# seanome/kmerseek

Measured on AMD Instinct MI355X. Metric: k-mers hashed+matched/sec, higher is better.
Workload: dtype u64

## Files before the change

include/kmerseek_amd.h:

```cpp
#ifndef KMERSEEK_AMD_H
#define KMERSEEK_AMD_H

#include <stddef.h>
#include <stdint.h>

#ifdef __cplusplus
extern "C" {
#endif

#define KS_ABI_VERSION 1

typedef enum ks_status {
    KS_OK = 0,
    KS_ERR_INVALID_MOLTYPE = 1,
    KS_ERR_INVALID_KSIZE = 2,
    KS_ERR_INVALID_RESIDUE = 3,
    KS_ERR_INVALID_ARG = 4,
    KS_ERR_OOM = 5,
    KS_ERR_HIP = 6,
    KS_ERR_NO_DEVICE = 7,
    KS_ERR_CAPACITY = 8,
    KS_ERR_INVALID_SCALED = 9
} ks_status;

typedef enum ks_moltype { KS_PROTEIN = 0, KS_DAYHOFF = 1, KS_HP = 2 } ks_moltype;

#define KS_SEED_DEFAULT 42ull
#define KS_MAX_KSIZE 128u

typedef struct ks_params {
    uint32_t ksize;
    uint32_t scaled;
    uint32_t moltype;
    uint32_t flags;
    uint64_t seed;
} ks_params;

typedef struct ks_ctx ks_ctx;
typedef struct ks_sketches ks_sketches;
typedef struct ks_index ks_index;
typedef struct ks_hits ks_hits;
typedef struct ks_kmerpos ks_kmerpos;
typedef struct ks_matchpos ks_matchpos;
typedef struct ks_regions ks_regions;
typedef struct ks_raligns ks_raligns;
typedef struct ks_cigars ks_cigars;
typedef struct ks_rscores ks_rscores;


uint32_t ks_abi_version(void);
const char *ks_status_string(int status);

int ks_moltype_from_string(const char *name, uint32_t *moltype_out);

uint64_t ks_max_hash(uint32_t scaled);

int ks_ctx_create(int device, void *hip_stream, ks_ctx **out);
void ks_ctx_destroy(ks_ctx *ctx);
const char *ks_last_error(const ks_ctx *ctx);
void *ks_ctx_stream(const ks_ctx *ctx);
int ks_ctx_synchronize(ks_ctx *ctx);
int ks_ctx_pool_stats(const ks_ctx *ctx, uint64_t *n_blocks, uint64_t *bytes_held, uint64_t *bytes_in_use,
                      uint64_t *n_mallocs);

int ks_ctx_sketch_stats(const ks_ctx *ctx, uint64_t out[4]);
int ks_ctx_search_stats(const ks_ctx *ctx, uint64_t out[5]);
int ks_ctx_fused_stats(const ks_ctx *ctx, uint64_t out[4]);
int ks_ctx_qfilter_stats(const ks_ctx *ctx, uint64_t out[2]);
int ks_ctx_reload_debug_env(ks_ctx *ctx);
int ks_debug_guard_selftest(const char *what);

int ks_dev_malloc(ks_ctx *ctx, uint64_t bytes, void **out);
int ks_dev_free(ks_ctx *ctx, void *ptr);
int ks_dev_upload(ks_ctx *ctx, void *dst_device, const void *src_host, uint64_t bytes);
int ks_dev_download(ks_ctx *ctx, void *dst_host, const void *src_device, uint64_t bytes);

int ks_host_alloc(ks_ctx *ctx, uint64_t bytes, void **out);
int ks_host_free(ks_ctx *ctx, void *ptr);


typedef struct ks_residue_error {
    uint32_t seq_index;
    uint32_t position;
    uint8_t residue;
} ks_residue_error;

int ks_validate_and_resolve(const uint8_t *seq, uint64_t len, int upper, uint64_t rng_seed,
                            uint8_t *out, uint64_t *out_len, ks_residue_error *err);


int ks_sketch_batch(ks_ctx *ctx, const uint8_t *residues, const uint64_t *seq_offsets,
                    uint32_t n_seqs, const ks_params *params, ks_sketches **out);

int ks_sketch_batch_device(ks_ctx *ctx, const uint8_t *d_residues, const uint64_t *d_seq_offsets,
                           uint32_t n_seqs, uint64_t n_residues, uint32_t max_seq_len,
                           const ks_params *params, ks_sketches **out);

int ks_sketch_queries_device(ks_ctx *ctx, const ks_index *index, const uint8_t *d_residues,
                             const uint64_t *d_seq_offsets, uint32_t n_seqs, uint64_t n_residues,
                             uint32_t max_seq_len, ks_sketches **out);

int ks_sketch_search_device(ks_ctx *ctx, const ks_index *index, const uint8_t *d_residues,
                            const uint64_t *d_seq_offsets, uint32_t n_seqs, uint64_t n_residues,
                            uint32_t max_seq_len, ks_sketches **sketches_out, ks_hits **hits_out);
int ks_sketch_search(ks_ctx *ctx, const ks_index *index, const uint8_t *residues, const uint64_t *seq_offsets,
                     uint32_t n_seqs, ks_sketches **sketches_out, ks_hits **hits_out);

uint32_t ks_sketches_n_seqs(const ks_sketches *s);
uint64_t ks_sketches_n_hashes(const ks_sketches *s);
uint64_t ks_sketches_n_windows(const ks_sketches *s);
int ks_sketches_has_postings(const ks_sketches *s);
void ks_sketches_params(const ks_sketches *s, ks_params *out);
const uint64_t *ks_sketches_device_offsets(const ks_sketches *s);
const uint64_t *ks_sketches_device_hashes(const ks_sketches *s);
const uint32_t *ks_sketches_device_abunds(const ks_sketches *s);
int ks_sketches_copy_to_host(ks_ctx *ctx, const ks_sketches *s, uint64_t *offsets,
                             uint64_t *hashes, uint32_t *abunds);
int ks_sketches_from_host(ks_ctx *ctx, const uint64_t *offsets, const uint64_t *hashes,
                          const uint32_t *abunds, uint32_t n_seqs, const ks_params *params,
                          ks_sketches **out);
int ks_sketches_union(ks_ctx *ctx, const ks_sketches *in, ks_sketches **out);
void ks_sketches_free(ks_sketches *s);


uint64_t ks_translate6_bound(uint64_t n_nt);
int ks_translate6_device(ks_ctx *ctx, const uint8_t *d_nt, const uint64_t *d_offsets, uint32_t n_seqs, uint64_t n_nt,
                         uint8_t *d_frames ,
                         uint64_t *d_frame_offsets , uint64_t *n_residues_out);
int ks_sketch_translated_device(ks_ctx *ctx, const uint8_t *d_nt, const uint64_t *d_offsets, uint32_t n_seqs, uint64_t n_nt,
                                uint32_t max_seq_len , const ks_params *params, ks_sketches **out);
int ks_sketch_translated(ks_ctx *ctx, const uint8_t *nt, const uint64_t *offsets, uint32_t n_seqs, const ks_params *params,
                         ks_sketches **out);
int ks_sketches_union_groups(ks_ctx *ctx, const ks_sketches *in, const uint32_t *group_offsets, uint32_t n_groups, ks_sketches **out);
uint32_t ks_debug_translate_chunk(void);
uint32_t ks_debug_union_rank_max(void);


#define KS_MASK_MAX_WINDOW 32
typedef struct ks_mask_opts { uint32_t window, k1_millibits, k2_millibits; } ks_mask_opts;
typedef struct ks_mask ks_mask;
typedef struct ks_segments ks_segments;
int ks_mask_device(ks_ctx *ctx, const uint8_t *d_residues, const uint64_t *d_seq_offsets, uint32_t n_seqs, uint64_t n_residues,
                   const ks_mask_opts *opts, ks_mask **out);
int ks_mask_batch(ks_ctx *ctx, const uint8_t *residues, const uint64_t *seq_offsets, uint32_t n_seqs, const ks_mask_opts *opts,
                  ks_mask **out);
uint32_t ks_mask_n_seqs(const ks_mask *m);
uint64_t ks_mask_n_residues(const ks_mask *m);
uint64_t ks_mask_n_masked(const ks_mask *m);
const uint8_t *ks_mask_device_mask(const ks_mask *m);
const uint32_t *ks_mask_device_masked_counts(const ks_mask *m);
int ks_mask_copy_to_host(ks_ctx *ctx, const ks_mask *m, uint8_t *mask, uint32_t *masked_counts);
void ks_mask_free(ks_mask *m);
int ks_mask_split_device(ks_ctx *ctx, const ks_mask *mask, const uint8_t *d_residues, const uint64_t *d_seq_offsets, uint32_t n_seqs,
                         uint64_t n_residues, uint32_t min_len, ks_segments **out);
uint64_t ks_segments_n_segs(const ks_segments *s);
uint64_t ks_segments_n_residues(const ks_segments *s);
uint32_t ks_segments_n_records(const ks_segments *s);
const uint32_t *ks_segments_device_seg_record(const ks_segments *s);
const uint32_t *ks_segments_device_seg_start(const ks_segments *s);
const uint64_t *ks_segments_device_seg_offsets(const ks_segments *s);
const uint8_t *ks_segments_device_residues(const ks_segments *s);
const uint32_t *ks_segments_device_group_offsets(const ks_segments *s);
int ks_segments_copy_to_host(ks_ctx *ctx, const ks_segments *s, uint32_t *seg_record, uint32_t *seg_start, uint64_t *seg_offsets,
                             uint8_t *residues, uint32_t *group_offsets);
void ks_segments_free(ks_segments *s);
int ks_sketch_masked_device(ks_ctx *ctx, const uint8_t *d_residues, const uint64_t *d_seq_offsets, uint32_t n_seqs, uint64_t n_residues,
                            uint32_t max_seq_len, const ks_params *params, const ks_mask_opts *opts, ks_sketches **out);
int ks_sketch_masked(ks_ctx *ctx, const uint8_t *residues, const uint64_t *seq_offsets, uint32_t n_seqs, const ks_params *params,
                     const ks_mask_opts *opts, ks_sketches **out);
int ks_kmer_positions_masked_device(ks_ctx *ctx, const uint8_t *d_residues, const uint64_t *d_seq_offsets, uint32_t n_seqs,
                                    uint64_t n_residues, const ks_params *params, const ks_mask_opts *opts, ks_kmerpos **out);
uint32_t ks_debug_mask_chunk(void);


int ks_kmer_positions(ks_ctx *ctx, const uint8_t *residues, const uint64_t *seq_offsets,
                      uint32_t n_seqs, const ks_params *params, ks_kmerpos **out);
int ks_kmer_positions_device(ks_ctx *ctx, const uint8_t *d_residues, const uint64_t *d_seq_offsets, uint32_t n_seqs,
                             uint64_t n_residues, const ks_params *params, ks_kmerpos **out);
uint64_t ks_kmerpos_count(const ks_kmerpos *p);
void ks_kmerpos_params(const ks_kmerpos *p, ks_params *out);
int ks_kmerpos_copy_to_host(ks_ctx *ctx, const ks_kmerpos *p, uint32_t *seq, uint32_t *start,
                            uint64_t *hash);
void ks_kmerpos_free(ks_kmerpos *p);


int ks_index_build(ks_ctx *ctx, const ks_sketches *targets, ks_index **out);
uint32_t ks_index_n_targets(const ks_index *ix);
uint64_t ks_index_n_postings(const ks_index *ix);
void ks_index_free(ks_index *ix);

int ks_search(ks_ctx *ctx, const ks_index *index, const ks_sketches *queries, ks_hits **out);
uint64_t ks_hits_count(const ks_hits *h);
uint64_t ks_hits_n_pair_instances(const ks_hits *h);
int ks_hits_partition_path(const ks_hits *h);
int ks_hits_bucket_posting_bytes(const ks_hits *h);
int ks_hits_copy_to_host(ks_ctx *ctx, const ks_hits *h, uint32_t *qid, uint32_t *tid,
                         uint32_t *intersect, uint64_t *n_weighted);
const uint32_t *ks_hits_device_qid(const ks_hits *h);
const uint32_t *ks_hits_device_tid(const ks_hits *h);
const uint32_t *ks_hits_device_intersect(const ks_hits *h);
const uint64_t *ks_hits_device_n_weighted(const ks_hits *h);
int ks_hits_copy_to_device(ks_ctx *ctx, const ks_hits *h, uint32_t qid_base, uint32_t tid_base, uint32_t *d_qid,
                           uint32_t *d_tid, uint32_t *d_intersect, uint64_t *d_n_weighted);
int ks_hits_pack64_to_device(ks_ctx *ctx, const ks_hits *h, uint32_t qid_base, uint32_t tid_base, int qbits, int tbits,
                             uint64_t *d_packed, uint32_t *d_esc_row, uint32_t *d_esc_intersect, uint64_t *d_esc_n_weighted,
                             uint32_t *d_n_esc, uint32_t esc_cap);
int ks_hits_unpack64_device(ks_ctx *ctx, const uint64_t *d_packed, uint64_t n, int qbits, int tbits, uint32_t *d_qid,
                            uint32_t *d_tid, uint32_t *d_intersect, uint64_t *d_n_weighted);
int ks_hits_merge_by_qid_device(ks_ctx *ctx, const uint32_t *d_qid, const uint32_t *d_tid, const uint32_t *d_intersect,
                                const uint64_t *d_n_weighted, const uint64_t *block_rows, uint32_t n_blocks, uint32_t n_queries,
                                uint32_t *d_out_qid, uint32_t *d_out_tid, uint32_t *d_out_intersect, uint64_t *d_out_n_weighted);
void ks_hits_free(ks_hits *h);


#define KS_SEARCH_ABUND_STATS 1u
typedef struct ks_search_opts {
    uint32_t flags;
    uint32_t reserved;
// ... 565 lines not shown
```

kmerseek_amd/_lib.py:

```python
from __future__ import annotations

import ctypes as C
import os
import sys

HERE = os.path.dirname(os.path.abspath(__file__))
SO_PATH = os.environ.get("KMERSEEK_AMD_LIB") or os.path.join(HERE, "libkmerseek_amd.so")

KS_OK = 0
KS_ERR_INVALID_MOLTYPE = 1
KS_ERR_INVALID_KSIZE = 2
KS_ERR_INVALID_RESIDUE = 3
KS_ERR_INVALID_ARG = 4
KS_ERR_OOM = 5
KS_ERR_HIP = 6
KS_ERR_NO_DEVICE = 7
KS_ERR_CAPACITY = 8
KS_ERR_INVALID_SCALED = 9

KS_PROTEIN, KS_DAYHOFF, KS_HP = 0, 1, 2
KS_SEED_DEFAULT = 42


class ks_params(C.Structure):
# ... 10 lines not shown

class ks_search_opts(C.Structure):
    _fields_ = [("flags", C.c_uint32), ("reserved", C.c_uint32), ("min_containment", C.c_double)]


class ks_matchpos_opts(C.Structure):
    _fields_ = [("flags", C.c_uint32), ("reserved", C.c_uint32), ("max_pairs", C.c_uint64)]


class ks_regions_opts(C.Structure):
    _fields_ = [("flags", C.c_uint32), ("min_kmers", C.c_uint32), ("max_gap", C.c_uint32), ("reserved", C.c_uint32)]


KS_RSCORE_ALPHABET = 28
KS_RSCORE_EXTEND = 1


class ks_rscore_opts(C.Structure):
    _fields_ = [("flags", C.c_uint32), ("x_drop", C.c_uint32), ("matrix", C.POINTER(C.c_int8)), ("reserved", C.c_uint64)]


KS_RALIGN_MAX_BAND = 31
KS_RALIGN_MAX_GAP_COST = 255
KS_RALIGN_MAX_X_DROP = 1 << 20


class ks_ralign_opts(C.Structure):
    _fields_ = [("matrix", C.POINTER(C.c_int8)), ("band", C.c_uint32), ("gap_open", C.c_uint32), ("gap_extend", C.c_uint32),
                ("x_drop", C.c_uint32), ("flags", C.c_uint32)]


KS_RTRACE_EQX = 1


class ks_rtrace_opts(C.Structure):
    _fields_ = [("flags", C.c_uint32), ("reserved", C.c_uint32), ("max_scratch_bytes", C.c_uint64)]


KS_RCULL_NONE = 0xFFFFFFFF
KS_RCULL_MIN_SCORE = 1


class ks_rcull_opts(C.Structure):
    _fields_ = [("overlap_pct", C.c_uint32), ("max_per_row", C.c_uint32), ("min_score", C.c_int64), ("flags", C.c_uint32),
                ("reserved", C.c_uint32)]


KS_RCHAIN_NONE = 0xFFFFFFFF


class ks_rchain_opts(C.Structure):
    _fields_ = [("max_gap", C.c_uint32), ("max_overlap", C.c_uint32), ("link_cost", C.c_uint32), ("skew_cost", C.c_uint32),
                ("overlap_cost", C.c_uint32), ("flags", C.c_uint32), ("reserved", C.c_uint32 * 2)]


KS_FFOLD_NONE = 0xFFFFFFFF


class ks_ffold_opts(C.Structure):
    _fields_ = [("flags", C.c_uint32), ("reserved", C.c_uint32 * 3)]


KS_RSTITCH_EQX = 1
KS_RSTITCH_MAX_FILL = 4096


class ks_rstitch_opts(C.Structure):
    _fields_ = [("max_fill", C.c_uint32), ("flags", C.c_uint32), ("max_scratch_bytes", C.c_uint64), ("reserved", C.c_uint32 * 2)]


KS_CIGAR_FSHIFT = 3
KS_FSTITCH_MAX_COST = 65536


class ks_fstitch_opts(C.Structure):
    _fields_ = [("max_fill", C.c_uint32), ("flags", C.c_uint32), ("frameshift_cost", C.c_uint32), ("reserved", C.c_uint32),
                ("max_scratch_bytes", C.c_uint64)]


KS_PILEUP_QUERY, KS_PILEUP_TARGET, KS_PILEUP_PROFILE = 0, 1, 1


class ks_pileup_opts(C.Structure):
    _fields_ = [("flags", C.c_uint32), ("side", C.c_uint32), ("reserved", C.c_uint64)]


KS_ASTATS_NO_COMPOSITION, KS_ASTATS_PAIRWISE, KS_ASTATS_ALLOW_UNGAPPED = 1, 2, 4
KS_ASTATS_ROW_REGULAR, KS_ASTATS_ROW_FALLBACK, KS_ASTATS_ROW_SKIPPED = 0, 1, 2
KS_ASTATS_MAX_SEQ_LEN = 1 << 20


class ks_astats_opts(C.Structure):
    _fields_ = [("flags", C.c_uint32), ("length_adjust", C.c_uint32), ("matrix", C.POINTER(C.c_int8)), ("lambda_", C.c_double),
                ("K", C.c_double), ("background", C.POINTER(C.c_double)), ("ratio_min", C.c_double), ("ratio_max", C.c_double),
                ("db_residues", C.c_uint64), ("db_seqs", C.c_uint64), ("reserved", C.c_uint64)]


class ks_signif_opts(C.Structure):
    _fields_ = [("flags", C.c_uint32), ("reserved", C.c_uint32)]


KS_BEST_INTERSECT, KS_BEST_TARGET_CONTAINMENT, KS_BEST_MAX_CONTAINMENT, KS_BEST_JACCARD, KS_BEST_SCORE = 0, 1, 2, 3, 4


class ks_best_opts(C.Structure):
    _fields_ = [("rank_by", C.c_uint32), ("k", C.c_uint32), ("flags", C.c_uint32), ("reserved", C.c_uint32)]


class ks_cluster_opts(C.Structure):
    _fields_ = [("similarity", C.c_uint32), ("n_nodes", C.c_uint32), ("threshold", C.c_double), ("flags", C.c_uint32),
                ("reserved", C.c_uint32)]


KS_GREEDY_ASSIGN_FIRST, KS_GREEDY_ASSIGN_BEST = 0, 1


class ks_greedy_opts(C.Structure):
    _fields_ = [("similarity", C.c_uint32), ("n_nodes", C.c_uint32), ("threshold", C.c_double), ("assign", C.c_uint32),
                ("flags", C.c_uint32)]


class ks_gather_opts(C.Structure):
    _fields_ = [("min_unique", C.c_uint32), ("max_results", C.c_uint32), ("flags", C.c_uint32), ("reserved", C.c_uint32)]


KS_MASK_MAX_WINDOW = 32


class ks_mask_opts(C.Structure):
    _fields_ = [("window", C.c_uint32), ("k1_millibits", C.c_uint32), ("k2_millibits", C.c_uint32)]


class ks_kernel_time(C.Structure):
    _fields_ = [("name", C.c_char * 48), ("launches", C.c_uint64), ("total_ms", C.c_double)]


_vp = C.c_void_p
_u8p = C.POINTER(C.c_uint8)
_u32p = C.POINTER(C.c_uint32)
_u64p = C.POINTER(C.c_uint64)
_pp = C.POINTER(C.c_void_p)
_parp = C.POINTER(ks_params)

SIGNATURES = {
    "ks_abi_version": (C.c_uint32, []),
    "ks_status_string": (C.c_char_p, [C.c_int]),
    "ks_moltype_from_string": (C.c_int, [C.c_char_p, _u32p]),
    "ks_max_hash": (C.c_uint64, [C.c_uint32]),
    "ks_ctx_create": (C.c_int, [C.c_int, _vp, _pp]),
    "ks_ctx_destroy": (None, [_vp]),
    "ks_last_error": (C.c_char_p, [_vp]),
    "ks_ctx_stream": (_vp, [_vp]),
    "ks_ctx_synchronize": (C.c_int, [_vp]),
    "ks_ctx_sketch_stats": (C.c_int, [_vp, C.POINTER(C.c_uint64 * 4)]),
    "ks_ctx_search_stats": (C.c_int, [_vp, C.POINTER(C.c_uint64 * 5)]),
    "ks_ctx_fused_stats": (C.c_int, [_vp, C.POINTER(C.c_uint64 * 4)]),
    "ks_ctx_qfilter_stats": (C.c_int, [_vp, C.POINTER(C.c_uint64 * 2)]),
    "ks_ctx_reload_debug_env": (C.c_int, [_vp]),
    "ks_debug_guard_selftest": (C.c_int, [C.c_char_p]),
    "ks_host_alloc": (C.c_int, [_vp, C.c_uint64, _pp]),
    "ks_host_free": (C.c_int, [_vp, _vp]),
    "ks_dev_malloc": (C.c_int, [_vp, C.c_uint64, _pp]),
    "ks_dev_free": (C.c_int, [_vp, _vp]),
    "ks_dev_upload": (C.c_int, [_vp, _vp, _vp, C.c_uint64]),
    "ks_dev_download": (C.c_int, [_vp, _vp, _vp, C.c_uint64]),
    "ks_ctx_pool_stats": (C.c_int, [_vp, _u64p, _u64p, _u64p, _u64p]),
    "ks_validate_and_resolve": (C.c_int, [C.c_char_p, C.c_uint64, C.c_int, C.c_uint64, C.c_char_p, _u64p,
                                          C.POINTER(ks_residue_error)]),
    "ks_sketch_batch": (C.c_int, [_vp, _vp, _vp, C.c_uint32, _parp, _pp]),
    "ks_sketch_batch_device": (C.c_int, [_vp, _vp, _vp, C.c_uint32, C.c_uint64, C.c_uint32, _parp, _pp]),
    "ks_sketch_queries_device": (C.c_int, [_vp, _vp, _vp, _vp, C.c_uint32, C.c_uint64, C.c_uint32, _pp]),
    "ks_sketch_search_device": (C.c_int, [_vp, _vp, _vp, _vp, C.c_uint32, C.c_uint64, C.c_uint32, _pp, _pp]),
    "ks_sketch_search": (C.c_int, [_vp, _vp, _vp, _vp, C.c_uint32, _pp, _pp]),
    "ks_sketches_has_postings": (C.c_int, [_vp]),
    "ks_sketches_n_seqs": (C.c_uint32, [_vp]),
    "ks_sketches_n_hashes": (C.c_uint64, [_vp]),
    "ks_sketches_n_windows": (C.c_uint64, [_vp]),
    "ks_sketches_params": (None, [_vp, _parp]),
    "ks_sketches_device_offsets": (_vp, [_vp]),
    "ks_sketches_device_hashes": (_vp, [_vp]),
    "ks_sketches_device_abunds": (_vp, [_vp]),
    "ks_sketches_copy_to_host": (C.c_int, [_vp, _vp, _vp, _vp, _vp]),
    "ks_sketches_from_host": (C.c_int, [_vp, _vp, _vp, _vp, C.c_uint32, _parp, _pp]),
    "ks_sketches_union": (C.c_int, [_vp, _vp, _pp]),
    "ks_sketches_free": (None, [_vp]),
    "ks_translate6_bound": (C.c_uint64, [C.c_uint64]),
    "ks_translate6_device": (C.c_int, [_vp, _vp, _vp, C.c_uint32, C.c_uint64, _vp, _vp, _u64p]),
    "ks_sketch_translated_device": (C.c_int, [_vp, _vp, _vp, C.c_uint32, C.c_uint64, C.c_uint32, _parp, _pp]),
    "ks_sketch_translated": (C.c_int, [_vp, _vp, _vp, C.c_uint32, _parp, _pp]),
    "ks_sketches_union_groups": (C.c_int, [_vp, _vp, _u32p, C.c_uint32, _pp]),
    "ks_debug_translate_chunk": (C.c_uint32, []),
    "ks_debug_union_rank_max": (C.c_uint32, []),
    "ks_mask_device": (C.c_int, [_vp, _vp, _vp, C.c_uint32, C.c_uint64, C.POINTER(ks_mask_opts), _pp]),
    "ks_mask_batch": (C.c_int, [_vp, _vp, _vp, C.c_uint32, C.POINTER(ks_mask_opts), _pp]),
    "ks_mask_n_seqs": (C.c_uint32, [_vp]),
    "ks_mask_n_residues": (C.c_uint64, [_vp]),
    "ks_mask_n_masked": (C.c_uint64, [_vp]),
    "ks_mask_device_mask": (_vp, [_vp]),
    "ks_mask_device_masked_counts": (_vp, [_vp]),
    "ks_mask_copy_to_host": (C.c_int, [_vp, _vp, _vp, _vp]),
    "ks_mask_free": (None, [_vp]),
    "ks_mask_split_device": (C.c_int, [_vp, _vp, _vp, _vp, C.c_uint32, C.c_uint64, C.c_uint32, _pp]),
    "ks_segments_n_segs": (C.c_uint64, [_vp]),
    "ks_segments_n_residues": (C.c_uint64, [_vp]),
    "ks_segments_n_records": (C.c_uint32, [_vp]),
    "ks_segments_device_seg_record": (_vp, [_vp]),
    "ks_segments_device_seg_start": (_vp, [_vp]),
    "ks_segments_device_seg_offsets": (_vp, [_vp]),
    "ks_segments_device_residues": (_vp, [_vp]),
    "ks_segments_device_group_offsets": (_vp, [_vp]),
    "ks_segments_copy_to_host": (C.c_int, [_vp, _vp, _vp, _vp, _vp, _vp, _vp]),
    "ks_segments_free": (None, [_vp]),
    "ks_sketch_masked_device": (C.c_int, [_vp, _vp, _vp, C.c_uint32, C.c_uint64, C.c_uint32, _parp, C.POINTER(ks_mask_opts), _pp]),
    "ks_sketch_masked": (C.c_int, [_vp, _vp, _vp, C.c_uint32, _parp, C.POINTER(ks_mask_opts), _pp]),
    "ks_kmer_positions_masked_device": (C.c_int, [_vp, _vp, _vp, C.c_uint32, C.c_uint64, _parp, C.POINTER(ks_mask_opts), _pp]),
    "ks_debug_mask_chunk": (C.c_uint32, []),
    "ks_kmer_positions": (C.c_int, [_vp, _vp, _vp, C.c_uint32, _parp, _pp]),
    "ks_kmer_positions_device": (C.c_int, [_vp, _vp, _vp, C.c_uint32, C.c_uint64, _parp, _pp]),
    "ks_kmerpos_count": (C.c_uint64, [_vp]),
    "ks_kmerpos_params": (None, [_vp, _parp]),
    "ks_kmerpos_copy_to_host": (C.c_int, [_vp, _vp, _vp, _vp, _vp]),
    "ks_kmerpos_free": (None, [_vp]),
    "ks_index_build": (C.c_int, [_vp, _vp, _pp]),
    "ks_index_n_targets": (C.c_uint32, [_vp]),
    "ks_index_n_postings": (C.c_uint64, [_vp]),
    "ks_index_free": (None, [_vp]),
    "ks_search": (C.c_int, [_vp, _vp, _vp, _pp]),
    "ks_hits_count": (C.c_uint64, [_vp]),
    "ks_hits_n_pair_instances": (C.c_uint64, [_vp]),
    "ks_hits_partition_path": (C.c_int, [_vp]),
    "ks_hits_bucket_posting_bytes": (C.c_int, [_vp]),
    "ks_hits_copy_to_host": (C.c_int, [_vp, _vp, _vp, _vp, _vp, _vp]),
    "ks_hits_device_qid": (_vp, [_vp]),
    "ks_hits_device_tid": (_vp, [_vp]),
    "ks_hits_device_intersect": (_vp, [_vp]),
    "ks_hits_device_n_weighted": (_vp, [_vp]),
    "ks_hits_copy_to_device": (C.c_int, [_vp, _vp, C.c_uint32, C.c_uint32, _vp, _vp, _vp, _vp]),
    "ks_hits_pack64_to_device": (C.c_int, [_vp, _vp, C.c_uint32, C.c_uint32, C.c_int, C.c_int, _vp, _vp, _vp, _vp, _vp, C.c_uint32]),
    "ks_hits_unpack64_device": (C.c_int, [_vp, _vp, C.c_uint64, C.c_int, C.c_int, _vp, _vp, _vp, _vp]),
    "ks_hits_merge_by_qid_device": (C.c_int, [_vp, _vp, _vp, _vp, _vp, C.POINTER(C.c_uint64), C.c_uint32, C.c_uint32, _vp, _vp, _vp, _vp]),
    "ks_hits_free": (None, [_vp]),
    "ks_search_ex": (C.c_int, [_vp, _vp, _vp, C.POINTER(ks_search_opts), _pp]),
    "ks_sketch_search_device_ex": (C.c_int, [_vp, _vp, _vp, _vp, C.c_uint32, C.c_uint64, C.c_uint32, C.POINTER(ks_search_opts), _pp,
                                             _pp]),
    "ks_sketch_search_ex": (C.c_int, [_vp, _vp, _vp, _vp, C.c_uint32, C.POINTER(ks_search_opts), _pp, _pp]),
    "ks_hits_has_abund_stats": (C.c_int, [_vp]),
    "ks_hits_device_median2": (_vp, [_vp]),
    "ks_hits_device_abund_ss": (_vp, [_vp]),
    "ks_hits_copy_abund_stats_to_host": (C.c_int, [_vp, _vp, _vp, _vp]),
    "ks_match_positions": (C.c_int, [_vp, _vp, _vp, _vp, C.POINTER(ks_matchpos_opts), _pp]),
    "ks_matchpos_n_rows": (C.c_uint64, [_vp]),
    "ks_matchpos_n_pairs": (C.c_uint64, [_vp]),
    "ks_matchpos_n_slices": (C.c_uint32, [_vp]),
    "ks_matchpos_device_row_offsets": (_vp, [_vp]),
    "ks_matchpos_device_q_start": (_vp, [_vp]),
    "ks_matchpos_device_t_start": (_vp, [_vp]),
    "ks_matchpos_device_q_lo": (_vp, [_vp]),
    "ks_matchpos_device_q_hi": (_vp, [_vp]),
    "ks_matchpos_device_t_lo": (_vp, [_vp]),
    "ks_matchpos_device_t_hi": (_vp, [_vp]),
    "ks_matchpos_copy_to_host": (C.c_int, [_vp, _vp, _vp, _vp, _vp, _vp, _vp, _vp, _vp]),
    "ks_matchpos_free": (None, [_vp]),
    "ks_match_regions": (C.c_int, [_vp, _vp, C.POINTER(ks_regions_opts), _pp]),
    "ks_regions_n_rows": (C.c_uint64, [_vp]),
    "ks_regions_n_regions": (C.c_uint64, [_vp]),
    "ks_regions_n_slices": (C.c_uint32, [_vp]),
    "ks_regions_device_row_offsets": (_vp, [_vp]),
    "ks_regions_device_q_start": (_vp, [_vp]),
    "ks_regions_device_t_start": (_vp, [_vp]),
    "ks_regions_device_length": (_vp, [_vp]),
    "ks_regions_device_n_kmers": (_vp, [_vp]),
    "ks_regions_device_covered": (_vp, [_vp]),
    "ks_regions_copy_to_host": (C.c_int, [_vp, _vp, _vp, _vp, _vp, _vp, _vp, _vp]),
    "ks_regions_free": (None, [_vp]),
    "ks_regions_score": (C.c_int, [_vp, _vp, _vp, _vp, _vp, C.c_uint32, C.c_uint64, _vp, _vp, C.c_uint32, C.c_uint64,
                                   C.POINTER(ks_rscore_opts), _pp]),
    "ks_rscores_n_rows": (C.c_uint64, [_vp]),
    "ks_rscores_n_regions": (C.c_uint64, [_vp]),
    "ks_rscores_device_row_offsets": (_vp, [_vp]),
    "ks_rscores_device_q_start": (_vp, [_vp]),
    "ks_rscores_device_t_start": (_vp, [_vp]),
    "ks_rscores_device_length": (_vp, [_vp]),
    "ks_rscores_device_score": (_vp, [_vp]),
    "ks_rscores_device_identities": (_vp, [_vp]),
    "ks_rscores_device_positives": (_vp, [_vp]),
    "ks_rscores_device_core_identities": (_vp, [_vp]),
    "ks_rscores_copy_to_host": (C.c_int, [_vp, _vp, _vp, _vp, _vp, _vp, _vp, _vp, _vp, _vp]),
    "ks_rscores_free": (None, [_vp]),
    "ks_debug_rscore_step": (C.c_uint32, []),
    "ks_regions_align": (C.c_int, [_vp, _vp, _vp, _vp, _vp, C.c_uint32, C.c_uint64, _vp, _vp, C.c_uint32, C.c_uint64,
                                   C.POINTER(ks_ralign_opts), _pp]),
    "ks_raligns_n_rows": (C.c_uint64, [_vp]),
    "ks_raligns_n_regions": (C.c_uint64, [_vp]),
    "ks_raligns_device_row_offsets": (_vp, [_vp]),
    "ks_raligns_device_q_start": (_vp, [_vp]),
    "ks_raligns_device_q_length": (_vp, [_vp]),
    "ks_raligns_device_t_start": (_vp, [_vp]),
    "ks_raligns_device_t_length": (_vp, [_vp]),
    "ks_raligns_device_score": (_vp, [_vp]),
    "ks_raligns_device_identities": (_vp, [_vp]),
    "ks_raligns_device_positives": (_vp, [_vp]),
    "ks_raligns_device_gap_opens": (_vp, [_vp]),
    "ks_raligns_device_gaps": (_vp, [_vp]),
    "ks_raligns_device_aln_length": (_vp, [_vp]),
    "ks_raligns_copy_to_host": (C.c_int, [_vp] * 13),
    "ks_raligns_free": (None, [_vp]),
    "ks_debug_ralign_chunk": (C.c_uint32, []),
# ... 262 lines not shown
```

kmerseek_amd/csrc/ks_common.h:

```cpp
#pragma once

#include <hip/hip_runtime.h>

#include <cstdint>
#include <cstdio>
#include <cstring>
#include <functional>
#include <initializer_list>
#include <new>
#include <stdexcept>
#include <string>
#include <vector>

#include "../../include/kmerseek_amd.h"

typedef uint8_t u8;
typedef uint16_t u16;
typedef uint32_t u32;
typedef uint64_t u64;
typedef int32_t i32;
typedef int64_t i64;

#define KS_WAVE 64

struct ks_pool_block {
    void *ptr;
    size_t size;
    bool in_use;
};

struct ks_timer_slot {
    hipEvent_t a, b;
    int name_id;
};

struct ks_copy_engine;

#define KS_DBG_LIST(X)                                                                                                   \
    X(STAGED_H2D) X(PLAIN_COPIES) X(PAIRS_LSD) X(MSD_LDS_CAP) X(SCAN_3PASS) X(INDEX_LSD) X(JOIN_FP) X(FP_COARSEN)        \
    X(PAIR_LIMIT) X(PBITS_MAX) X(RECORD_BITS) X(ONE_CURSOR) X(JOIN_SEGS) X(JOIN_SEG_CAP) X(JOIN_SPARSE)                \
    X(NO_ROWS_HINT) X(ROWS_TICKET) X(FORCE_ROWS_TICKET_RETRY) X(FORCE_TICKET_RETRY) X(NO_PLAN) X(NO_COMPACT) X(SPAN)      \
    X(NO_PACK) X(PLAN_SYNC) X(TILE_R) X(OUT_CAP) X(POOL_CAP) X(THROW) X(QCAP) X(LOOKBACK_SKIP) X(SYNC_API) X(POSTINGS12) X(POSTINGS10) X(NO_DEFER) X(BUCKET) X(JOIN_SPLIT) X(SUBSHIFT) X(MATCHPOS_ROW_BITS) X(SIGNIF_WAVE_ROWS) X(BEST_PATH) X(REGIONS_ROW_BITS) X(QFILTER) X(QFILTER_OCC) X(CLUSTER_PATH) X(GATHER_PATH) X(GREEDY_PATH) X(UNION_PATH) X(AGG_CAP) X(ROWS_PATH) X(CULL_PATH) X(CHAIN_PATH) X(COMP_PATH) X(PILEUP_PATH)
enum ks_dbg_id {
#define KS_DBG_ENUM(n) KS_DBG_##n,
    KS_DBG_LIST(KS_DBG_ENUM)
#undef KS_DBG_ENUM
    KS_DBG_COUNT
};
struct ks_debug {
    bool set[KS_DBG_COUNT];
    char val[KS_DBG_COUNT][32];
};
void ks_debug_load(ks_debug *d);

struct ks_ctx {
    int device = 0;
    ks_copy_engine *copy = nullptr;
    hipStream_t stream = nullptr;
    bool own_stream = false;
    int n_cus = 256;
    ks_debug dbg;
    u64 pool_cap = 0;
    std::string err;
    std::vector<ks_pool_block> pool;
    u64 pool_mallocs = 0;
    int timing = 0;
    std::vector<std::string> t_names;
    std::vector<u64> t_launches;
    std::vector<double> t_ms;
    std::vector<ks_timer_slot> t_pending;
    std::vector<std::pair<hipEvent_t, hipEvent_t>> t_free;
    bool t_open = false;
    u64 *h_pin = nullptr;
    u64 pair_cap_hint = 0;
    u64 rows_hint = 0;
    bool sketch_use_ticket = false;
    u64 sketch_ticket_fallbacks = 0, sketch_compact_fallbacks = 0, sketch_cap_fallbacks = 0;
    bool rows_use_ticket = false; u64 rows_ticket_fallbacks = 0;
    u64 fused_deferred = 0, fused_redos = 0;
    u64 fused_aggregated = 0;
    u64 join_retries = 0;
    double rows_mult = 0.0;
    u64 agg_used = 0, agg_overflows = 0, agg_oflow_rows = 0;
    bool qfilter_pays = true;
    u64 qfilter_seen = 0, qfilter_dropped = 0;
    u64 qf_last_seen = 0, qf_last_kept = 0;
    u64 join_table = 0, fused_table_joined = 0;
    unsigned long long *scan_ring = nullptr;
    u32 *scan_ticket = nullptr;
    u32 scan_ticket_base = 0;
    u8 *d_lut = nullptr;
    unsigned long long *h_flag = nullptr;
    unsigned long long wait_seq = 0;
};

int ks_stream_wait(ks_ctx *ctx);
#define KS_FETCH_MAX 4
struct ks_fetch_seg {
    const void *src;
    u32 *dst;
    u32 rows, row_words, src_stride;
};
static inline ks_fetch_seg ks_fetch_words(const void *src, void *dst, u32 n_words32) { return ks_fetch_seg{src, (u32 *)dst, 1u, n_words32, n_words32}; }
int ks_stream_wait_fetch(ks_ctx *ctx, const ks_fetch_seg *segs, int n);

void *ks_pool_alloc(ks_ctx *ctx, size_t bytes);
void ks_pool_free(ks_ctx *ctx, void *ptr);
void ks_pool_trim(ks_ctx *ctx);

int ks_fail(ks_ctx *ctx, int status, const char *fmt, ...);
static inline const char *ks_dbg(const ks_ctx *ctx, int id) { return (ctx && ctx->dbg.set[id]) ? ctx->dbg.val[id] : nullptr; }

int ks_guard_fail(ks_ctx *ctx, int status, const char *what) noexcept;
void ks_guard_enter(ks_ctx *ctx);
template <typename F>
static inline int ks_guard(ks_ctx *ctx, F &&body) noexcept {
    try {
        ks_guard_enter(ctx);
        return body();
    } catch (const std::bad_alloc &) {
        return ks_guard_fail(ctx, KS_ERR_OOM, "out of host memory (std::bad_alloc)");
    } catch (const std::exception &e) {
        return ks_guard_fail(ctx, KS_ERR_HIP, e.what());
    } catch (...) {
        return ks_guard_fail(ctx, KS_ERR_HIP, "unknown exception");
    }
}

void ks_timer_begin(ks_ctx *ctx, const char *name);
void ks_timer_end(ks_ctx *ctx);

#define KS_HIP(ctx, expr)                                                                          \
    do {                                                                                           \
        hipError_t e__ = (expr);                                                                   \
        if (e__ != hipSuccess)                                                                     \
            return ks_fail(ctx, KS_ERR_HIP, "%s failed: %s (%s:%d)", #expr, hipGetErrorString(e__), \
                           __FILE__, __LINE__);                                                    \
    } while (0)

#define KS_TRY(expr)                        \
    do {                                    \
        int s__ = (expr);                   \
        if (s__ != KS_OK) return s__;       \
    } while (0)

#define KS_LAUNCH(ctx, name, kernel, grid, block, ...)                                   \
    do {                                                                                 \
        ks_timer_begin(ctx, name);                                                       \
        hipLaunchKernelGGL(kernel, dim3(grid), dim3(block), 0, (ctx)->stream, __VA_ARGS__); \
        ks_timer_end(ctx);                                                               \
        KS_HIP(ctx, hipGetLastError());                                                  \
    } while (0)

template <typename T>
static inline int ks_alloc(ks_ctx *ctx, T **out, size_t count) {
    void *p = ks_pool_alloc(ctx, (count ? count : 1) * sizeof(T));
    if (!p) return KS_ERR_OOM;
    *out = (T *)p;
    return KS_OK;
}

struct ks_scratch {
    ks_ctx *ctx;
    void *blk[16];
    int n = 0;
    explicit ks_scratch(ks_ctx *c) : ctx(c) {}
    ks_scratch(const ks_scratch &) = delete;
    ~ks_scratch() { for (int i = 0; i < n; i++) ks_pool_free(ctx, blk[i]); }
    template <typename T> int alloc(T **out, size_t count) {
        if (n == 16) return ks_fail(ctx, KS_ERR_HIP, "internal error: scratch table full");
        KS_TRY(ks_alloc(ctx, out, count));
        blk[n++] = *out;
        return KS_OK;
    }
    void free(void *p) { if (forget(p)) ks_pool_free(ctx, p); }
    template <typename T> T *keep(T *p) { forget(p); return p; }
    bool forget(void *p) {
        for (int i = 0; p && i < n; i++)
            if (blk[i] == p) { blk[i] = blk[--n]; return true; }
        return false;
    }
};

struct ks_ctl {
    u64 *dev = nullptr;
    u64 *host = nullptr;
    u32 n_words = 0;
    int init(ks_ctx *ctx, ks_scratch &sc, u32 pin_slot, u32 n_bad, u32 n_count) {
        n_words = n_bad + n_count;
        host = ctx->h_pin + pin_slot;
        KS_TRY(sc.alloc(&dev, n_words));
        KS_HIP(ctx, hipMemsetAsync(dev, 0xff, n_bad * sizeof(u64), ctx->stream));
        KS_HIP(ctx, hipMemsetAsync(dev + n_bad, 0, n_count * sizeof(u64), ctx->stream));
        return KS_OK;
    }
    unsigned long long *words() const { return (unsigned long long *)dev; }
    u32 *low32(u32 i) const { return (u32 *)(dev + i); }
    ks_fetch_seg fetch() const { return ks_fetch_words(dev, host, 2 * n_words); }
    u64 operator[](u32 i) const { return host[i]; }
    bool bad(u32 i) const { return host[i] != ~0ULL; }
};

template <typename T>
struct ks_result {
    T *obj = nullptr;
    T **out;
    void (*free_fn)(T *);
    ks_result(ks_ctx *ctx, T **out_, void (*f)(T *)) : out(out_), free_fn(f) {
        *out = nullptr;
        obj = new T();
        obj->ctx = ctx;
    }
    ks_result(const ks_result &) = delete;
    ~ks_result() {
        if (!obj) return;
        (void)hipStreamSynchronize(obj->ctx->stream);
        free_fn(obj);
    }
    T *operator->() const { return obj; }
    operator T *() const { return obj; }
    int commit() { *out = obj; obj = nullptr; return KS_OK; }
};

struct ks_column { void *dst; const void *src; size_t bytes; };
int ks_copy_d2h(ks_ctx *ctx, void *dst_host, const void *src_device, size_t bytes);
static inline int ks_columns_to_host(ks_ctx *ctx, const ks_column *cols, size_t n) {
    KS_HIP(ctx, hipSetDevice(ctx->device));
    for (const ks_column *c = cols; c < cols + n; c++)
        if (c->dst && c->bytes) KS_TRY(ks_copy_d2h(ctx, c->dst, c->src, c->bytes));
    KS_HIP(ctx, hipStreamSynchronize(ctx->stream));
// ... 602 lines not shown
```

kmerseek_amd/csrc/ks_ctx.hip:

```cpp
#include <cstdarg>
#include <algorithm>

#include "ks_common.h"

int ks_fail(ks_ctx *ctx, int status, const char *fmt, ...) {
    char buf[512];
    va_list ap;
    va_start(ap, fmt);
    vsnprintf(buf, sizeof buf, fmt, ap);
    va_end(ap);
    if (ctx) {
        try { ctx->err = buf; } catch (...) { }
    }
    return status;
}

extern "C" uint32_t ks_abi_version(void) { return KS_ABI_VERSION; }


bool ks_same_params(const ks_params &a, const ks_params &b) {
    return a.ksize == b.ksize && a.scaled == b.scaled && a.moltype == b.moltype && a.seed == b.seed && a.flags == b.flags;
}
int ks_params_check_same(ks_ctx *ctx, const char *pass, const char *noun, const ks_params &a, const ks_params &b) {
    if (ks_same_params(a, b)) return KS_OK;
// ... 18 lines not shown
}

static void build_luts(u8 *lut) {
    for (int m = 0; m < 3; m++)
        for (int b = 0; b < 256; b++) {
            u8 c = (b >= 'a' && b <= 'z') ? (u8)(b - 32) : (u8)b;
            u8 e = c;
            if (m == KS_DAYHOFF) {
                switch (c) {
                case 'C': e = 'a'; break;
                case 'A': case 'G': case 'P': case 'S': case 'T': e = 'b'; break;
                case 'D': case 'E': case 'N': case 'Q': e = 'c'; break;
                case 'H': case 'K': case 'R': e = 'd'; break;
                case 'I': case 'L': case 'M': case 'V': e = 'e'; break;
                case 'F': case 'W': case 'Y': e = 'f'; break;
                default: e = 'X';
                }
            } else if (m == KS_HP) {
                switch (c) {
                case 'A': case 'F': case 'G': case 'I': case 'L': case 'M': case 'P': case 'V':
                case 'W': case 'Y': e = 'h'; break;
                case 'N': case 'C': case 'S': case 'T': case 'D': case 'E': case 'R': case 'H':
                case 'K': case 'Q': e = 'p'; break;
                default: e = 'X';
                }
            }
            lut[m * 256 + b] = e;
        }
}

void ks_debug_load(ks_debug *d) {
    static const char *const names[KS_DBG_COUNT] = {
#define KS_DBG_NAME(n) "KS_DEBUG_" #n,
        KS_DBG_LIST(KS_DBG_NAME)
#undef KS_DBG_NAME
    };
    for (int i = 0; i < KS_DBG_COUNT; i++) {
        const char *v = getenv(names[i]);
        d->set[i] = v != nullptr;
        d->val[i][0] = 0;
        if (v) { strncpy(d->val[i], v, sizeof d->val[i] - 1); d->val[i][sizeof d->val[i] - 1] = 0; }
    }
}
static void debug_apply(ks_ctx *ctx) {
    ks_debug_load(&ctx->dbg);
    const char *cap = ks_dbg(ctx, KS_DBG_POOL_CAP);
    ctx->pool_cap = cap ? strtoull(cap, nullptr, 10) : 0;
}
extern "C" int ks_ctx_reload_debug_env(ks_ctx *ctx) {
    if (!ctx) return KS_ERR_INVALID_ARG;
    debug_apply(ctx);
    return KS_OK;
}

int ks_guard_fail(ks_ctx *ctx, int status, const char *what) noexcept {
    if (ctx) {
        try {
            ctx->err.assign(status == KS_ERR_OOM ? "" : "internal error: ");
            ctx->err.append(what ? what : "?");
        } catch (...) {
        }
    }
    return status;
}
void ks_guard_enter(ks_ctx *ctx) {
    const char *t = ks_dbg(ctx, KS_DBG_THROW);
    if (!t) return;
    if (!strcmp(t, "bad_alloc")) throw std::bad_alloc();
    if (!strcmp(t, "runtime")) throw std::runtime_error("KS_DEBUG_THROW");
    if (!strcmp(t, "other")) throw 42;
}

extern "C" int ks_debug_guard_selftest(const char *what) {
    return ks_guard(nullptr, [&]() -> int {
        if (what && !strcmp(what, "bad_alloc")) { std::vector<char> v; v.reserve((size_t)-1 / 2); }
        if (what && !strcmp(what, "runtime")) throw std::runtime_error("selftest");
        if (what && !strcmp(what, "other")) throw 42;
        return KS_OK;
    });
}

extern "C" int ks_ctx_create(int device, void *hip_stream, ks_ctx **out) {
    if (!out) return KS_ERR_INVALID_ARG;
    *out = nullptr;
    int n = 0;
    if (hipGetDeviceCount(&n) != hipSuccess || n <= 0) return KS_ERR_NO_DEVICE;
    if (device < 0 || device >= n) return KS_ERR_INVALID_ARG;
    ks_ctx *ctx = new (std::nothrow) ks_ctx();
    if (!ctx) return KS_ERR_OOM;
    ctx->device = device;
    try { ctx->err.reserve(640); ctx->pool.reserve(256); } catch (...) { delete ctx; return KS_ERR_OOM; }
    debug_apply(ctx);
    if (hipSetDevice(device) != hipSuccess) { delete ctx; return KS_ERR_HIP; }
    hipDeviceProp_t prop;
    if (hipGetDeviceProperties(&prop, device) == hipSuccess) ctx->n_cus = prop.multiProcessorCount;
    if (hip_stream) {
        ctx->stream = (hipStream_t)hip_stream;
    } else {
        if (hipStreamCreateWithFlags(&ctx->stream, hipStreamNonBlocking) != hipSuccess) { delete ctx; return KS_ERR_HIP; }
        ctx->own_stream = true;
    }
    if (hipHostMalloc((void **)&ctx->h_pin, KS_PIN_WORDS * sizeof(u64), hipHostMallocCoherent) != hipSuccess) { delete ctx; return KS_ERR_HIP; }
    if (hipHostMalloc((void **)&ctx->h_flag, 64, hipHostMallocCoherent) != hipSuccess) { (void)hipGetLastError(); ctx->h_flag = nullptr; }
    else *ctx->h_flag = 0;
    if (hipMalloc((void **)&ctx->d_lut, 3 * 256) != hipSuccess) { delete ctx; return KS_ERR_OOM; }
    u8 lut[768];
    build_luts(lut);
    if (hipMemcpy(ctx->d_lut, lut, sizeof lut, hipMemcpyHostToDevice) != hipSuccess) { delete ctx; return KS_ERR_HIP; }
    *out = ctx;
    return KS_OK;
}

extern "C" void ks_ctx_destroy(ks_ctx *ctx) {
    if (!ctx) return;
    (void)hipSetDevice(ctx->device);
    (void)hipStreamSynchronize(ctx->stream);
    ks_copy_engine_destroy(ctx);
    for (auto &t : ctx->t_pending) { (void)hipEventDestroy(t.a); (void)hipEventDestroy(t.b); }
    for (auto &t : ctx->t_free) { (void)hipEventDestroy(t.first); (void)hipEventDestroy(t.second); }
    for (auto &b : ctx->pool) (void)hipFree(b.ptr);
    if (ctx->d_lut) (void)hipFree(ctx->d_lut);
    if (ctx->h_pin) (void)hipHostFree(ctx->h_pin);
    if (ctx->h_flag) (void)hipHostFree(ctx->h_flag);
    if (ctx->scan_ring) (void)hipFree(ctx->scan_ring);
    if (ctx->scan_ticket) (void)hipFree(ctx->scan_ticket);
    if (ctx->own_stream) (void)hipStreamDestroy(ctx->stream);
    delete ctx;
}

extern "C" const char *ks_last_error(const ks_ctx *ctx) { return ctx ? ctx->err.c_str() : "no context"; }
extern "C" void *ks_ctx_stream(const ks_ctx *ctx) { return ctx ? (void *)ctx->stream : nullptr; }
extern "C" int ks_ctx_synchronize(ks_ctx *ctx) {
    return ks_guard(ctx, [&]() -> int {
    if (!ctx) return KS_ERR_INVALID_ARG;
    KS_HIP(ctx, hipStreamSynchronize(ctx->stream));
    return KS_OK;
    });
}

extern "C" int ks_ctx_pool_stats(const ks_ctx *ctx, uint64_t *n_blocks, uint64_t *bytes_held, uint64_t *bytes_in_use,
                                 uint64_t *n_mallocs) {
    return ks_guard((ks_ctx *)ctx, [&]() -> int {
    if (!ctx) return KS_ERR_INVALID_ARG;
    u64 held = 0, used = 0;
    for (auto &b : ctx->pool) { held += b.size; if (b.in_use) used += b.size; }
    if (n_blocks) *n_blocks = ctx->pool.size();
    if (bytes_held) *bytes_held = held;
    if (bytes_in_use) *bytes_in_use = used;
    if (n_mallocs) *n_mallocs = ctx->pool_mallocs;
    return KS_OK;
    });
}

extern "C" int ks_ctx_sketch_stats(const ks_ctx *ctx, uint64_t out[4]) {
    return ks_guard((ks_ctx *)ctx, [&]() -> int {
    if (!ctx || !out) return KS_ERR_INVALID_ARG;
    out[0] = ctx->sketch_ticket_fallbacks; out[1] = ctx->sketch_use_ticket ? 1 : 0;
    out[2] = ctx->sketch_compact_fallbacks; out[3] = ctx->sketch_cap_fallbacks;
    return KS_OK;
    });
}

extern "C" int ks_ctx_search_stats(const ks_ctx *ctx, uint64_t out[5]) {
    return ks_guard((ks_ctx *)ctx, [&]() -> int {
    if (!ctx || !out) return KS_ERR_INVALID_ARG;
    out[0] = ctx->join_retries; out[1] = ctx->rows_ticket_fallbacks;
    out[2] = ctx->agg_used; out[3] = ctx->agg_overflows;
    out[4] = ctx->join_table;
    return KS_OK;
    });
}

extern "C" int ks_ctx_qfilter_stats(const ks_ctx *ctx, uint64_t out[2]) {
    return ks_guard((ks_ctx *)ctx, [&]() -> int {
    if (!ctx || !out) return KS_ERR_INVALID_ARG;
    out[0] = ctx->qfilter_seen; out[1] = ctx->qfilter_dropped;
    return KS_OK;
    });
}

extern "C" int ks_ctx_fused_stats(const ks_ctx *ctx, uint64_t out[4]) {
    return ks_guard((ks_ctx *)ctx, [&]() -> int {
    if (!ctx || !out) return KS_ERR_INVALID_ARG;
    out[0] = ctx->fused_deferred; out[1] = ctx->fused_redos; out[2] = ctx->fused_aggregated;
    out[3] = ctx->fused_table_joined;
    return KS_OK;
    });
}

extern "C" int ks_dev_malloc(ks_ctx *ctx, uint64_t bytes, void **out) {
    return ks_guard(ctx, [&]() -> int {
    if (!ctx || !out) return KS_ERR_INVALID_ARG;
    KS_HIP(ctx, hipSetDevice(ctx->device));
    if (hipMalloc(out, bytes ? bytes : 256) != hipSuccess) { (void)hipGetLastError(); return ks_fail(ctx, KS_ERR_OOM, "hipMalloc(%llu) failed", (unsigned long long)bytes); }
    return KS_OK;
    });
}
extern "C" int ks_dev_free(ks_ctx *ctx, void *ptr) {
    return ks_guard(ctx, [&]() -> int {
    if (!ctx) return KS_ERR_INVALID_ARG;
    KS_HIP(ctx, hipStreamSynchronize(ctx->stream));
    KS_HIP(ctx, hipFree(ptr));
    return KS_OK;
    });
}
extern "C" int ks_dev_upload(ks_ctx *ctx, void *dst, const void *src, uint64_t bytes) {
    return ks_guard(ctx, [&]() -> int {
    if (!ctx || (bytes && (!dst || !src))) return KS_ERR_INVALID_ARG;
    KS_HIP(ctx, hipSetDevice(ctx->device));
    KS_TRY(ks_copy_h2d(ctx, dst, src, (size_t)bytes));
    KS_HIP(ctx, hipStreamSynchronize(ctx->stream));
    return KS_OK;
    });
}
extern "C" int ks_dev_download(ks_ctx *ctx, void *dst, const void *src, uint64_t bytes) {
    return ks_guard(ctx, [&]() -> int {
    if (!ctx || (bytes && (!dst || !src))) return KS_ERR_INVALID_ARG;
    KS_HIP(ctx, hipSetDevice(ctx->device));
    KS_TRY(ks_copy_d2h(ctx, dst, src, (size_t)bytes));
    KS_HIP(ctx, hipStreamSynchronize(ctx->stream));
    return KS_OK;
    });
}

__global__ void k_host_stamp(unsigned long long *flag, unsigned long long seq) {
    __hip_atomic_store(flag, seq, __ATOMIC_RELEASE, __HIP_MEMORY_SCOPE_SYSTEM);
}
struct ks_fetch_args { ks_fetch_seg seg[KS_FETCH_MAX]; int n; };
__global__ __launch_bounds__(256) void k_host_report(ks_fetch_args F, unsigned long long *flag, unsigned long long seq) {
    for (int s = 0; s < F.n; s++) {
        const ks_fetch_seg g = F.seg[s];
        const u32 total = g.rows * g.row_words;
        for (u32 i = threadIdx.x; i < total; i += blockDim.x) {
            const u32 r = i / g.row_words, c = i - r * g.row_words;
            const u32 v = __hip_atomic_load((const u32 *)g.src + (size_t)r * g.src_stride + c, __ATOMIC_RELAXED, __HIP_MEMORY_SCOPE_AGENT);
            __hip_atomic_store(g.dst + i, v, __ATOMIC_RELAXED, __HIP_MEMORY_SCOPE_SYSTEM);
        }
    }
    __threadfence_system();
    __syncthreads();
    if (threadIdx.x == 0) __hip_atomic_store(flag, seq, __ATOMIC_RELEASE, __HIP_MEMORY_SCOPE_SYSTEM);
}

static int stream_wait_poll(ks_ctx *ctx, unsigned long long seq);

int ks_stream_wait_fetch(ks_ctx *ctx, const ks_fetch_seg *segs, int n) {
    if (n > KS_FETCH_MAX) return ks_fail(ctx, KS_ERR_INVALID_ARG, "too many fetch segments");
    if (!ctx->h_flag || ks_dbg(ctx, KS_DBG_SYNC_API)) {
        for (int i = 0; i < n; i++) {
            const ks_fetch_seg &g = segs[i];
            if (g.rows == 1 || g.src_stride == g.row_words)
                KS_HIP(ctx, hipMemcpyAsync(g.dst, g.src, (size_t)g.rows * g.row_words * sizeof(u32), hipMemcpyDeviceToHost, ctx->stream));
            else
                KS_HIP(ctx, hipMemcpy2DAsync(g.dst, (size_t)g.row_words * sizeof(u32), g.src, (size_t)g.src_stride * sizeof(u32),
                                            (size_t)g.row_words * sizeof(u32), g.rows, hipMemcpyDeviceToHost, ctx->stream));
        }
        KS_HIP(ctx, hipStreamSynchronize(ctx->stream));
        return KS_OK;
    }
    ks_fetch_args F;
    memset(&F, 0, sizeof F);
    for (int i = 0; i < n; i++) F.seg[i] = segs[i];
    F.n = n;
    const unsigned long long seq = ++ctx->wait_seq;
    hipLaunchKernelGGL(k_host_report, dim3(1), dim3(256), 0, ctx->stream, F, ctx->h_flag, seq);
    if (hipGetLastError() != hipSuccess) return ks_fail(ctx, KS_ERR_HIP, "k_host_report launch failed");
    return stream_wait_poll(ctx, seq);
}

int ks_stream_wait(ks_ctx *ctx) {
    if (!ctx->h_flag || ks_dbg(ctx, KS_DBG_SYNC_API)) {
        KS_HIP(ctx, hipStreamSynchronize(ctx->stream));
        return KS_OK;
    }
    const unsigned long long seq = ++ctx->wait_seq;
    hipLaunchKernelGGL(k_host_stamp, dim3(1), dim3(1), 0, ctx->stream, ctx->h_flag, seq);
    if (hipGetLastError() != hipSuccess) { KS_HIP(ctx, hipStreamSynchronize(ctx->stream)); return KS_OK; }
    return stream_wait_poll(ctx, seq);
}

static int stream_wait_poll(ks_ctx *ctx, unsigned long long seq) {
    for (unsigned spins = 1;; spins++) {
        if (__atomic_load_n(ctx->h_flag, __ATOMIC_ACQUIRE) == seq) return KS_OK;
        if ((spins & 0xfffu) == 0) {
            const hipError_t q = hipStreamQuery(ctx->stream);
            if (q == hipSuccess) {
                if (__atomic_load_n(ctx->h_flag, __ATOMIC_ACQUIRE) == seq) return KS_OK;
                KS_HIP(ctx, hipStreamSynchronize(ctx->stream));
                return KS_OK;
            }
            if (q != hipErrorNotReady) return ks_fail(ctx, KS_ERR_HIP, "stream failed: %s", hipGetErrorString(q));
            if (spins > (1u << 26)) { KS_HIP(ctx, hipStreamSynchronize(ctx->stream)); return KS_OK; }
        }
#if defined(__x86_64__)
        __builtin_ia32_pause();
#endif
    }
}

static size_t pool_class(size_t bytes) {
    if (bytes <= 4096) return (bytes + 255) & ~(size_t)255;
    const int e = 63 - __builtin_clzll((unsigned long long)(bytes - 1));
    const size_t step = (size_t)1 << (e - 2);
    return (bytes + step - 1) & ~(step - 1);
}

void *ks_pool_alloc(ks_ctx *ctx, size_t bytes) {
    if (bytes == 0) bytes = 256;
    const size_t want = pool_class(bytes);
    for (size_t i = 0; i < ctx->pool.size(); i++) {
        auto &b = ctx->pool[i];
// ... 239 lines not shown
```

kmerseek_amd/csrc/ks_sketch.hip:

```cpp
#include "ks_tile.h"

#define SK_MED_MAX (SK_TILE - 16)
#define SK_NR 8
static const u32 sk_r_cand_host[SK_NR] = {2544, 2800, 3056, 3312, 3568, 3824, 3952, 4016};
#ifndef SK_MINW
#define SK_MINW 6
#endif
#define SK_NFLAG (SK_TILE / 32)
#ifndef SK_LB_WAVES
#define SK_LB_WAVES 1
#endif
#define SK_C3MAX 32u
#define SK_QB_CAP 128u

#ifdef SK_STAMP
#define SK_STAMP_SLOTS 4096
__device__ unsigned long long sk_stamp_acc[SK_STAMP_SLOTS][16];
#define SK_STAMP_AT(i) do { if (threadIdx.x == 0) { unsigned long long t_ = clock64(); \
    atomicAdd(&sk_stamp_acc[blockIdx.x % SK_STAMP_SLOTS][i], t_ - sk_t_prev); sk_t_prev = clock64(); } } while (0)
extern "C" void ks_debug_read_stamps(unsigned long long *out, int reset) {
    static unsigned long long host[SK_STAMP_SLOTS][16];
    (void)hipMemcpyFromSymbol(host, HIP_SYMBOL(sk_stamp_acc), sizeof host);
    for (int i = 0; i < 16; i++) { out[i] = 0; for (int s = 0; s < SK_STAMP_SLOTS; s++) out[i] += host[s][i]; }
    if (reset) { memset(host, 0, sizeof host); (void)hipMemcpyToSymbol(HIP_SYMBOL(sk_stamp_acc), host, sizeof host); }
}
#elif defined(SK_STOP_AFTER)
#define SK_STAMP_AT(i) do { if ((i) == SK_STOP_AFTER) return; } while (0)
#else
#define SK_STAMP_AT(i) do { } while (0)
#endif

KS_DEV bool sk_deferred(u64 start, u64 len, u32 R, u32 span) { return start % R + len > span - 16; }
KS_DEV u32 sk_div(u32 x, u32 d, u32 rcp) { return d == 1 ? x : __umulhi(x, rcp); }

KS_DEV u32 sk_wave_totals_scan(const u32 *smem, u32 lane, u32 wave_u , u32 *total) {
    constexpr u32 NW = SK_THREADS / 64;
    static_assert(NW <= 16, "one DPP row");
    u32 v = lane < NW ? smem[lane] : 0u;
    v += (u32)__builtin_amdgcn_update_dpp(0, (int)v, 0x111, 0xf, 0xf, true);
    v += (u32)__builtin_amdgcn_update_dpp(0, (int)v, 0x112, 0xf, 0xf, true);
    v += (u32)__builtin_amdgcn_update_dpp(0, (int)v, 0x114, 0xf, 0xf, true);
    if (NW > 8) v += (u32)__builtin_amdgcn_update_dpp(0, (int)v, 0x118, 0xf, 0xf, true);
    *total = (u32)__builtin_amdgcn_readlane((int)v, NW - 1);
    return wave_u ? (u32)__builtin_amdgcn_readlane((int)v, (int)wave_u - 1) : 0u;
}
KS_DEV u32 sk_block_excl_scan2(u32 a, u32 b, u32 *smem, u32 *total_a, u32 *excl_b) {
    const u32 lane = threadIdx.x & 63, wave = threadIdx.x >> 6;
    constexpr u32 NW = SK_THREADS / 64;
    const u32 ia = ks_wave_incl_scan(a), ib = ks_wave_incl_scan(b);
    if (lane == 63) { smem[wave] = ia; smem[NW + 1 + wave] = ib; }
    __syncthreads();
    const u32 wave_u = (u32)__builtin_amdgcn_readfirstlane((int)wave);
    u32 tot_b;
    const u32 base_a = sk_wave_totals_scan(smem, lane, wave_u, total_a);
    const u32 base_b = sk_wave_totals_scan(smem + NW + 1, lane, wave_u, &tot_b);
    *excl_b = base_b + ib - b;
    if (threadIdx.x == 0) smem[NW] = tot_b;
    return base_a + ia - a;
}

KS_DEV u32 sk_block_excl_scan1(u32 a, u32 *smem) {
    const u32 lane = threadIdx.x & 63, wave = threadIdx.x >> 6;
    const u32 ia = ks_wave_incl_scan(a);
    if (lane == 63) smem[wave] = ia;
    __syncthreads();
    u32 total;
    const u32 base = sk_wave_totals_scan(smem, lane, (u32)__builtin_amdgcn_readfirstlane((int)wave), &total);
    return base + ia - a;
}

KS_DEV u32 sk_digit(u64 h, u32 K, u32 kshift, u32 mask) {
    const u32 hi = (u32)(h >> 32);
    return (kshift ? (hi >> kshift) : __umulhi(hi, K)) & mask;
}

enum : u32 {
    SK_CTL_WINDOWS = 0, SK_CTL_MAX_LEN = 1,
    SK_CTL_N_PK_LONG = 2,
    SK_CTL_MED = 4, SK_CTL_LONG = 4 + SK_NR,
    SK_CTL_TICKET = 20,
    SK_CTL_CLS = 21,
    SK_CTL_PK_TILES = 22,
    SK_CTL_TOTAL = 23,
    SK_CTL_DROPS = 24,
    SK_CTL_LB_ROUNDS = 25,
    SK_CTL_DROPS_DEF = 26,
    SK_CTL_WORDS = 32,
    SK_CTL_CURSORS = SK_CTL_WORDS, SK_CTL_CURSOR_WORDS = 1024,
    SK_CTL_TILE_STATUS = SK_CTL_CURSORS + SK_CTL_CURSOR_WORDS,
};
static_assert(SK_CTL_LONG + SK_NR <= SK_CTL_TICKET && SK_CTL_LB_ROUNDS < SK_CTL_WORDS && SK_CTL_DROPS_DEF < SK_CTL_WORDS,
              "sketch control block layout");
static_assert(SK_CTL_WORDS <= KS_PIN_SKETCH_WORDS && SK_CTL_WORDS <= KS_PIN_SKETCH_SYNC_WORDS, "pinned slots of the sketch read-back");
enum : u32 { SK_ST_LOOKBACK = 1u, SK_ST_POSTINGS = 2u, SK_ST_COMPACT = 4u };
#define SK_BO_B(x) (((x) >> 12) & 0xfffu)
#define SK_BO_O(x) ((x) & 0xfffu)
#define SK_BO_S(x) ((x) >> 24)

struct sk_bounds {
    const u32 *loff;
    const u64 *goff;
    u64 g0;
    u32 s_first;
    bool in_lds;
    KS_DEV u32 at(u32 s) const {
        if (in_lds) return loff[s - s_first];
        u64 v = goff[s] - g0;
        return v > 0x7fffffffULL ? 0x7fffffffu : (u32)v;
    }
};

struct sk_seq {
    u32 s;
    u32 ls, le;
    u32 nw;
    u32 mul;
    bool ok;
};

KS_DEV void sk_load_seq(sk_seq &q, const sk_args &A, const sk_bounds &B, u32 s_end) {
    if (q.s >= s_end) { q.ok = false; q.ls = 0xffffffffu; q.le = 0xffffffffu; q.nw = 0; q.mul = 0; return; }
    q.ls = B.at(q.s);
    q.le = B.at(q.s + 1);
    const u32 len = q.le - q.ls;
    q.nw = (len >= A.k && q.le <= A.le_cap && len <= A.max_len_tile) ? (len - A.k + 1) : 0;
    q.mul = sk_bucket_mul(q.nw, A.sfix);
    q.ok = q.nw > 0;
}

KS_DEV u32 sk_place_window(const sk_args &A, u32 p, u64 h, sk_seq &q, const sk_bounds &B, u32 s_end, u32 *cnt) {
    while (q.s < s_end && p >= q.le) { q.s++; sk_load_seq(q, A, B, s_end); }
    const bool keep = q.ok && p >= q.ls && p + A.k <= q.le && h != 0 && h <= A.max_hash;
    u32 bo = 0xffffffffu;
    if (keep) {
        const u32 b = q.ls + __umulhi((u32)(h >> 32), q.mul);
        const u32 sh = (b & 1u) * 16u;
        const u32 o = (atomicAdd(&cnt[b >> 1], 1u << sh) >> sh) & 0xffffu;
        const u32 srel = q.s - B.s_first;
        bo = ((srel < 254u ? srel : 254u) << 24) | (b << 12) | o;
    }
    return bo;
}


#define PK_CHUNK 1024
#define PK_MAX_LEN (SK_MED_MAX - 16)

__global__ __launch_bounds__(64) void k_pack_walk(const u64 *offs, u32 n_seqs, u32 chunk ,
                                                  u32 *chunk_tiles , u32 *chunk_cnt) {
    __shared__ u64 lo_s[PK_CHUNK + 1];
    const u32 lane = threadIdx.x;
    const u32 c0 = blockIdx.x * chunk;
    const u32 n = (n_seqs - c0) < chunk ? (n_seqs - c0) : chunk;
    for (u32 i = lane; i <= n; i += 64) lo_s[i] = offs[c0 + i];
    __builtin_amdgcn_wave_barrier();
    u32 s = 0, nt = 0;
    while (s < n) {
        const u64 limit = (lo_s[s] & ~15ULL) + SK_MED_MAX;
        u32 lo = s, hi = n + 1;
        while (hi - lo > 1) {
            const u32 step = (hi - lo + 63) / 64;
            const u32 idx = lo + (lane + 1) * step;
            const bool ok = idx < hi && lo_s[idx] <= limit;
            const u64 m = __ballot(ok);
            const u32 good = m == ~0ULL ? 64u : (u32)__builtin_ctzll(~m);
            const u32 nlo = lo + good * step;
            const u32 nhi = lo + (good + 1) * step;
            lo = nlo < hi ? nlo : hi - 1;
            hi = nhi < hi ? nhi : hi;
        }
        u32 e = lo;
        if (e == s) e = s + 1;
        else if (e < n && lo_s[e + 1] - lo_s[e] > PK_MAX_LEN) e++;
        if (lane == 0) chunk_tiles[c0 + nt] = c0 + s;
        nt++;
        s = e;
    }
    if (lane == 0) chunk_cnt[blockIdx.x] = nt;
}

__global__ __launch_bounds__(256) void k_pack_fill(const u64 *offs, u32 n_seqs, u32 chunk, const u32 *chunk_tiles, const u32 *chunk_cnt, u32 n_chunks,
                                                   u32 *tile_first, u64 *tile_g0, u32 *n_tiles_out) {
    __shared__ u32 scan_smem[256 / 64 + 1];
    u32 part = 0;
    for (u32 c = threadIdx.x; c < blockIdx.x; c += 256) part += chunk_cnt[c];
    u32 total;
    (void)ks_block_excl_scan(part, scan_smem, &total);
    const u32 base = total, mine = chunk_cnt[blockIdx.x];
    for (u32 i = threadIdx.x; i < mine; i += 256) {
        const u32 sf = chunk_tiles[blockIdx.x * chunk + i];
        tile_first[base + i] = sf;
        tile_g0[base + i] = offs[sf] & ~15ULL;
    }
    if (blockIdx.x == n_chunks - 1 && threadIdx.x == 0) {
        tile_first[base + mine] = n_seqs;
        *n_tiles_out = base + mine;
    }
}

__global__ __launch_bounds__(256) void k_tile_plan(const u64 *offs, u32 n_seqs, u32 n_tiles, u32 R, u32 *tile_first) {
    const u32 t = blockIdx.x * blockDim.x + threadIdx.x;
    if (t > n_tiles) return;
    tile_first[t] = t == n_tiles ? n_seqs : ks_lower_bound_u64(offs, n_seqs, (u64)t * R);
}

template <int H, int NW, int KC>
KS_DEV void sk_cmp_half(const sk_args &A, const sk_bounds &B, sk_seq &q, const u64 *wl, u32 p0, bool active, u32 s_first, u32 s_end,
                        u32 lane, u64 *hlist, u8 *slist, u32 *cursor) {
    static_assert(NW == 4 || NW == 8, "a half or the whole of a thread's windows");
    u64 h[NW];
    u32 keep = 0, sr[2] = {0, 0};
    if (active) {
        sk_hash_windows<H, NW, KC>(h, wl, A.k, A.seed);
        if ((KC ? (u32)KC : A.k) >= SK_E) {
            const u32 srel = q.s - s_first;
#pragma unroll
            for (int i = 0; i < NW; i++)
                if ((p0 + H + i - q.ls) < q.nw && h[i] != 0 && h[i] <= A.max_hash) keep |= 1u << i;
            sr[0] = sr[1] = srel * 0x01010101u;
        } else {
#pragma unroll
            for (int i = 0; i < NW; i++) {
                const u32 p = p0 + H + i;
                while (q.s < s_end && p >= q.le) { q.s++; sk_load_seq(q, A, B, s_end); }
                if (q.ok && p >= q.ls && p + A.k <= q.le && h[i] != 0 && h[i] <= A.max_hash) {
                    keep |= 1u << i;
                    sr[i >> 2] |= (q.s - s_first) << (8 * (i & 3));
                }
            }
        }
    }
    const u32 nk = (u32)__popc(keep);
    const u32 incl = ks_wave_incl_scan(nk);
    const u32 wtot = (u32)__builtin_amdgcn_readlane((int)incl, 63);
    u32 wbase = 0;
    if (wtot) {
        if (lane == 0) wbase = atomicAdd(cursor, wtot);
        wbase = (u32)__builtin_amdgcn_readfirstlane((int)wbase);
    }
    u32 pos = wbase + incl - nk;
#pragma unroll
    for (int i = 0; i < NW; i++)
        if (keep & (1u << i)) {
            if (pos < SK_TILE) {
                hlist[pos] = h[i];
                slist[pos] = (u8)(sr[i >> 2] >> (8 * (i & 3)));
            }
            pos++;
        }
}

template <int MODE, int CMP, int KC>
KS_DEV void sk_tile_body(const sk_args &A, const u32 tile_in) {
    static_assert(!(CMP && MODE), "the compacting variant is for shared tiles");
    __shared__ __attribute__((aligned(16))) u64 res_w[(SK_TILE + SK_PAD) / 8];
    __shared__ __attribute__((aligned(16))) u32 cnt[SK_TILE / 2 + 4];
    __shared__ __attribute__((aligned(8))) u16 dseq[SK_SEQ_CAP + 2];
    __shared__ u16 dsd[SK_SEQ_CAP + 2];
    __shared__ __attribute__((aligned(16))) u64 tmp[SK_TILE];
    __shared__ u32 flagbits[SK_NFLAG];
    __shared__ u32 flagpre[SK_NFLAG + 1];
    __shared__ u32 scan_smem[2 * (SK_THREADS / 64 + 1)];
    __shared__ u32 loff[SK_SEQ_CAP + 2];
    __shared__ u8 lut_s[256];
#ifdef SK_LDS_PAD
    __shared__ u32 lds_pad[SK_LDS_PAD / 4];
    if (threadIdx.x == 0 && A.n_res == 0xfffffffffffffffULL) lds_pad[A.k] = 1;
#endif
    __shared__ u32 bins[256 + 1];
    __shared__ unsigned long long gaddr[256];

    const u32 tid = threadIdx.x;
    u8 *res_b = (u8 *)res_w;
#ifdef SK_STAMP
    unsigned long long sk_t_prev = clock64();
#endif

    __shared__ u32 tile_s;
    __shared__ u32 ext_n;
    __shared__ u32 ndup_s;
    __shared__ u32 ext_seq[4], ext_cnt[4], ext_d[4];
    __shared__ unsigned long long lb_sum[SK_THREADS / 64];
    __shared__ u32 lb_pre[SK_THREADS / 64];
    u32 tile = tile_in;
    constexpr u32 NCH = (SK_TILE + SK_PAD) / 16;
    static_assert(NCH <= SK_THREADS, "one staging chunk per thread");
    u32 ticket_v = 0;
    if (MODE == 0 && tid == 0) ticket_v = A.use_ticket ? atomicAdd(&A.ticket[0], 1u) : tile_in;
    u32 lut_v = 0;
    if (!A.upper_only && tid < 256) lut_v = A.lut[tid];
    if (tid < 256) bins[tid] = 0;
    if (tid == 256) bins[256] = 0;
    static_assert(SK_TILE / 2 == SK_THREADS * 4, "one 16-byte store per thread zeroes the bucket counters");
    *(uint4 *)&cnt[tid * 4u] = make_uint4(0, 0, 0, 0);
    if (tid < 4) cnt[SK_TILE / 2 + tid] = 0;
    if (tid < SK_NFLAG) flagbits[tid] = 0;
    __shared__ u32 n_list_s;
    if (tid == 0) { ext_n = 0; n_list_s = 0; ndup_s = 0; }
    if (MODE == 0 && A.use_ticket) {
        if (tid == 0) tile_s = ticket_v;
        __syncthreads();
        tile = tile_s;
    }
    uint4 rv = make_uint4(0, 0, 0, 0);
    const bool packed = MODE == 0 && !CMP && A.R == 0;
    tile = (u32)__builtin_amdgcn_readfirstlane((int)tile);
    u64 g0p = 0;
    if (packed) g0p = A.tile_g0[tile];
    u32 s_first, s_end;
    if (MODE == 1) { s_first = A.seq_list[tile]; s_end = s_first + 1; }
    else { s_first = A.seq_list[tile]; s_end = A.seq_list[tile + 1]; }
    if (!A.upper_only && tid < 256) lut_s[tid] = (u8)lut_v;
    if (MODE == 0 && tid < NCH) rv = sk_load16(A.res, A.n_res, (packed ? g0p : (u64)tile * A.R) + (u64)tid * 16);
    if (s_first >= s_end) {
        if (MODE == 0 && tid == 0)
            __hip_atomic_store(&A.tile_status[tile], KS_LB_AGG | 0ULL, __ATOMIC_RELAXED, __HIP_MEMORY_SCOPE_AGENT);
        return;
    }
    const u64 g0 = MODE == 0 ? (packed ? g0p : (u64)tile * A.R) : (A.offs[s_first] & ~15ULL);
    const u32 ns = s_end - s_first;
    sk_bounds B;
    B.loff = loff; B.goff = A.offs; B.g0 = g0; B.s_first = s_first; B.in_lds = ns <= SK_SEQ_CAP;
    if (B.in_lds)
        for (u32 i = tid; i <= ns; i += SK_THREADS) {
            u64 v = A.offs[s_first + i] - g0;
            loff[i] = v > 0x7fffffffULL ? 0x7fffffffu : (u32)v;
        }

    SK_STAMP_AT(0);
    if (MODE == 1) {
        u64 span_end = A.offs[s_end];
        if (span_end > g0 + SK_TILE) span_end = g0 + SK_TILE;
        if (tid < NCH) {
            const u64 g = g0 + (u64)tid * 16;
            if (g < span_end) rv = sk_load16(A.res, A.n_res, g);
        }
        __syncthreads();
    }
    if (MODE == 0 && !A.upper_only) __syncthreads();
    if (tid < NCH) *(uint4 *)(res_b + (size_t)tid * 16) = sk_encode16(rv, lut_s, A.upper_only);
    __syncthreads();

    SK_STAMP_AT(1);
    const u32 q0 = tid * SK_E;
    sk_seq q;
    const u32 kk = KC ? (u32)KC : A.k;
    const bool onerun = kk >= SK_E;
    {
        q.s = sk_seq_beyond(s_first, s_end, onerun ? q0 + kk - 1u : q0, [&](u32 s) { return B.at(s + 1); });
        sk_load_seq(q, A, B, s_end);
    }
    const u64 *wl = res_w + tid;
    u64 h[SK_E];
    u32 bo[SK_E];
#ifdef SK_NO_EARLY
    const bool early = false;
#else
    const bool early = !CMP && A.part_keys != nullptr && B.in_lds;
#endif
    u32 rkp[SK_E / 2] = {0, 0, 0, 0};
    u32 kept_mask = 0, srel_one = 0;
    if (CMP) {
        u8 *slist = (u8 *)cnt;
        const u32 lane = tid & 63u;
        u32 end_l = B.at(s_end);
        if (end_l > A.span) end_l = A.span;
        const u32 n_sub = B.in_lds ? (end_l + SK_TILE - 1) / SK_TILE : 0;
        for (u32 sub = 0; sub < n_sub; sub++) {
            if (sub > 0) {
                if (tid < NCH) *(uint4 *)(res_b + (size_t)tid * 16) = sk_encode16(rv, lut_s, A.upper_only);
                __syncthreads();
            }
            SK_STAMP_AT(9);
            if (sub + 1 < n_sub && tid < NCH)
                rv = sk_load16(A.res, A.n_res, (u64)tile * A.R + (u64)(sub + 1) * SK_TILE + (u64)tid * 16);
            const u32 p0 = sub * SK_TILE + q0;
            const bool active = p0 < end_l;
            if (active) {
                q.s = sk_seq_beyond(s_first, s_end, onerun ? p0 + kk - 1u : p0, [&](u32 s) { return B.at(s + 1); });
                sk_load_seq(q, A, B, s_end);
            }
            if constexpr (KC == 16) {
                sk_cmp_half<0, 8, KC>(A, B, q, wl, p0, active, s_first, s_end, lane, tmp, slist, &n_list_s);
            } else {
                sk_cmp_half<0, 4, KC>(A, B, q, wl, p0, active, s_first, s_end, lane, tmp, slist, &n_list_s);
                sk_cmp_half<4, 4, KC>(A, B, q, wl, p0, active, s_first, s_end, lane, tmp, slist, &n_list_s);
            }
            SK_STAMP_AT(10);
            __syncthreads();
            SK_STAMP_AT(11);
        }
        const u32 n_list = n_list_s;
        if (!B.in_lds || n_list > SK_TILE) {
            if (tid == 0) {
                atomicOr(&A.ticket[1], 4u);
                __hip_atomic_store(&A.tile_status[tile], (tile == 0 ? KS_LB_PRE : KS_LB_AGG) | 0ULL, __ATOMIC_RELAXED,
                                   __HIP_MEMORY_SCOPE_AGENT);
            }
            return;
        }
        u32 srl[SK_E];
#pragma unroll
        for (int i = 0; i < SK_E; i++) {
            const u32 idx = (u32)i * SK_THREADS + tid;
            const bool live = idx < n_list;
            h[i] = live ? tmp[idx] : 0;
            srl[i] = live ? (u32)slist[idx] : 0xffffffffu;
        }
        __syncthreads();
        for (u32 i = tid; i < SK_TILE / 2 + 4; i += SK_THREADS) cnt[i] = 0;
        uint2 *stab = (uint2 *)res_w;
        for (u32 i = tid; i < ns; i += SK_THREADS) {
            const u32 ls = loff[i], le = loff[i + 1], len = le - ls;
            const u32 nw = (len >= A.k && le <= A.le_cap) ? len - A.k + 1 : 0;
            const u32 nb = sk_div(nw + A.c_div - 1, A.c_div, A.c_rcp);
            stab[i] = make_uint2(sk_div(ls, A.c_div, A.c_rcp) + i, sk_bucket_mul(nb, A.sfix));
        }
        __syncthreads();
#pragma unroll
        for (int i = 0; i < SK_E; i++) {
            bo[i] = 0xffffffffu;
            if (srl[i] != 0xffffffffu) {
                const uint2 t = stab[srl[i]];
                const u32 b = t.x + __umulhi((u32)(h[i] >> 32), t.y);
                const u32 sh = (b & 1u) * 16u;
                const u32 o = (atomicAdd(&cnt[b >> 1], 1u << sh) >> sh) & 0xffffu;
                bo[i] = (srl[i] << 24) | (b << 12) | o;
            }
        }
    } else
    if (q0 < B.at(s_end)) {
        sk_hash_windows<0, SK_E, KC>(h, wl, A.k, A.seed);
        if (onerun) {
            const u32 srel = q.s - B.s_first;
            const u32 s24 = (srel < 254u ? srel : 254u) << 24;
            const bool thr = A.max_hash != ~0ULL;
            u32 bb[SK_E], rt[SK_E];
            u32 kpm = 0;
#pragma unroll
            for (int i = 0; i < SK_E; i++) {
                bool keep = (q0 + (u32)i - q.ls) < q.nw && h[i] != 0;
                if (thr) keep = keep && h[i] <= A.max_hash;
                kpm |= keep ? (1u << i) : 0u;
                const u32 b = q.ls + __umulhi((u32)(h[i] >> 32), q.mul);
                bb[i] = keep ? b : (u32)SK_TILE + 2u;
            }
#pragma unroll
            for (int i = 0; i < SK_E; i++)
                rt[i] = atomicAdd(&cnt[bb[i] >> 1], ((kpm >> i) & 1u) << ((bb[i] << 4) & 31u));
#pragma unroll
            for (int i = 0; i < SK_E; i++)
                bo[i] = ((kpm >> i) & 1u) ? (s24 | (bb[i] << 12) | __builtin_amdgcn_ubfe(rt[i], bb[i] << 4, 16u)) : 0xffffffffu;
            kept_mask = kpm; srel_one = s24 >> 24;
        } else {
#pragma unroll
            for (int i = 0; i < SK_E; i++) bo[i] = sk_place_window(A, q0 + i, h[i], q, B, s_end, cnt);
        }
        if (early) {
            if (A.part_kshift) {
                u32 rr[SK_E];
#pragma unroll
                for (int i = 0; i < SK_E; i++) {
                    const bool kept = bo[i] != 0xffffffffu;
                    rr[i] = atomicAdd(&bins[kept ? (((u32)(h[i] >> 32) >> A.part_kshift) & A.part_mask) : 256u], kept ? 1u : 0u);
                }
#pragma unroll
                for (int i = 0; i < SK_E; i++) rkp[i >> 1] |= (bo[i] != 0xffffffffu ? rr[i] : 0u) << ((i & 1) * 16);
            } else {
#pragma unroll
                for (int i = 0; i < SK_E; i++)
                    if (bo[i] != 0xffffffffu)
                        rkp[i >> 1] |= atomicAdd(&bins[__umulhi((u32)(h[i] >> 32), A.part_K) & A.part_mask], 1u) << ((i & 1) * 16);
            }
        }
    } else {
#pragma unroll
        for (int i = 0; i < SK_E; i++) { h[i] = 0; bo[i] = 0xffffffffu; }
    }
    __syncthreads();

    SK_STAMP_AT(2);
    if (MODE == 0) {
        for (u32 s = s_first + tid; s < s_end; s += SK_THREADS) {
            const u32 ls = B.at(s), le = B.at(s + 1);
            if (le > A.le_cap || le - ls > A.max_len_tile) {
                const u32 e = atomicAdd(&ext_n, 1u);
                if (e < 4) { ext_seq[e] = s; ext_cnt[e] = A.kept[s]; ext_d[e] = 0; }
            }
        }
    }
    const u32 q_skip = CMP ? 2u * (ns < SK_SEQ_CAP + 1u ? ns : SK_SEQ_CAP + 1u) : 0u;
    u16 *qb = (u16 *)((u32 *)res_w + q_skip);
    u16 *q3 = qb + SK_QB_CAP;
    const u32 q_ents = ((SK_TILE + SK_PAD) / 4 - q_skip) * 2 - SK_QB_CAP;
    u32 q3cap = q_ents;
    if (A.debug_qcap) q3cap = q3cap < A.debug_qcap ? q3cap : A.debug_qcap;
    u32 ovf = 0;
    u32 pairs = 0;
    {
        const uint4 w4 = *(const uint4 *)&cnt[q0 >> 1];
        const u32 w[4] = {w4.x, w4.y, w4.z, w4.w};
        const u32 hs = w[0] + w[1] + w[2] + w[3];
        const u32 s = (hs & 0xffffu) + (hs >> 16);
        u32 ge2 = 0, ge3 = 0, big = 0;
#pragma unroll
        for (int j = 0; j < 4; j++) {
            ge2 |= (((w[j] + 0x7ffe7ffeu) & 0x80008000u) >> 15) << j;
            ge3 |= (((w[j] + 0x7ffd7ffdu) & 0x80008000u) >> 15) << j;
        }
        if (s > SK_C3MAX) {
#pragma unroll
            for (int j = 0; j < 4; j++) big |= (((w[j] + (0x8000u - SK_C3MAX - 1u) * 0x00010001u) & 0x80008000u) >> 15) << j;
        }
        u32 m2 = ge2 & ~ge3, m3 = ge3 & ~big;
        pairs = m2;
        const u32 code = ((u32)__popc(m3) << 12) | ((u32)__popc(big) << 24);
        u32 total, at;
        u32 ex = sk_block_excl_scan2(s, code, scan_smem, &total, &at);
        u32 i3 = (at >> 12) & 0xfffu, ib = at >> 24;
        u32 o[4];
#pragma unroll
        for (int j = 0; j < 4; j++) {
            const u32 lo = w[j] & 0xffffu;
            o[j] = ex | ((ex + lo) << 16);
            ex += lo + (w[j] >> 16);
        }
        *(uint4 *)&cnt[q0 >> 1] = make_uint4(o[0], o[1], o[2], o[3]);
        if (tid == SK_THREADS - 1) cnt[SK_TILE / 2] = total | (total << 16);
        while (m3) {
            const u32 bit = (u32)__builtin_ctz(m3);
            m3 &= m3 - 1u;
            if (i3 < q3cap) q3[i3] = (u16)(q0 + 2u * (bit & 15u) + (bit >> 4)); else ovf |= 1u << bit;
            i3++;
        }
        while (big) {
            const u32 bit = (u32)__builtin_ctz(big);
            big &= big - 1u;
            qb[ib++] = (u16)(q0 + 2u * (bit & 15u) + (bit >> 4));
        }
    }
    __syncthreads();
    auto bstart = [&](u32 b) -> u32 { return ((const u16 *)cnt)[b]; };
    const u32 n_kept = bstart(SK_TILE);
    const u32 ne = MODE == 0 ? (ext_n < 4 ? ext_n : 4) : 0;
    u64 agg = n_kept;
    for (u32 e = 0; e < ne; e++) agg += ext_cnt[e];
    if (MODE == 0 && tid == 0 && tile != A.debug_skip_tile)
        __hip_atomic_store(&A.tile_status[tile], (tile == 0 ? KS_LB_PRE : KS_LB_AGG) | agg, __ATOMIC_RELAXED, __HIP_MEMORY_SCOPE_AGENT);

    SK_STAMP_AT(3);
    {
        u32 st8[SK_E];
#pragma unroll
        for (int i = 0; i < SK_E; i++) st8[i] = bstart(SK_BO_B(bo[i]));
#pragma unroll
        for (int i = 0; i < SK_E; i++)
            if (bo[i] != 0xffffffffu) tmp[st8[i] + SK_BO_O(bo[i])] = h[i];
    }
    if (B.in_lds) {
        for (u32 i = tid; i <= ns; i += SK_THREADS)
            dseq[i] = (u16)(i == ns ? n_kept : bstart(CMP ? ((const uint2 *)res_w)[i].x : loff[i]));
    } else {
        for (u32 s = s_first + tid; s < s_end; s += SK_THREADS) {
            const u32 ls = B.at(s);
            const u32 d = ls <= SK_TILE ? bstart(ls) : n_kept;
            if (d < n_kept) atomicOr(&flagbits[d >> 5], 1u << (d & 31));
        }
    }
    __syncthreads();

    SK_STAMP_AT(4);
    u32 nd = 0;
    auto sort_small = [&](u32 sb, u32 c) {
        for (u32 a = 1; a < c; a++) {
            const u64 x = tmp[sb + a];
            u32 j = a;
            while (j > 0) {
                const u64 y = tmp[sb + j - 1];
                if (y <= x) { nd += y == x ? 1u : 0u; break; }
                tmp[sb + j] = y;
                j--;
            }
            if (j != a) tmp[sb + j] = x;
        }
    };
    {
        const u32 qc = scan_smem[SK_THREADS / 64];
        const u32 n3 = ((qc >> 12) & 0xfffu) < q3cap ? ((qc >> 12) & 0xfffu) : q3cap;
        const u32 nb = qc >> 24;
        {
            const uint4 st4 = *(const uint4 *)&cnt[q0 >> 1];
            const u32 st[4] = {st4.x, st4.y, st4.z, st4.w};
#pragma unroll
            for (int j = 0; j < 4; j++) {
                const u32 stj = st[j];
#pragma unroll
                for (int hh = 0; hh < 2; hh++)
                    if (pairs & (1u << (j + 16 * hh))) {
                        const u32 sb = hh ? stj >> 16 : stj & 0xffffu;
                        const u64 x = tmp[sb], y = tmp[sb + 1];
                        if (x > y) { tmp[sb] = y; tmp[sb + 1] = x; }
                        nd += x == y ? 1u : 0u;
                    }
            }
        }
        for (u32 e = SK_THREADS - 1u - tid; e < n3; e += SK_THREADS) {
            const u32 b = q3[e], sb = bstart(b);
            sort_small(sb, bstart(b + 1) - sb);
        }
        while (ovf) {
            const u32 bit = (u32)__builtin_ctz(ovf);
            ovf &= ovf - 1u;
            const u32 b = q0 + 2u * (bit & 15u) + (bit >> 4), sb = bstart(b);
            sort_small(sb, bstart(b + 1) - sb);
        }
        if (nb) {
            for (u32 e = 0; e < nb; e++) {
                const u32 b = qb[e], sb = bstart(b), c = bstart(b + 1) - sb;
                u64 xs[SK_E];
                u32 rkb[SK_E];
#pragma unroll
                for (int i = 0; i < SK_E; i++) {
                    const u32 j = (u32)i * SK_THREADS + tid;
                    rkb[i] = 0xffffffffu;
                    if (j < c) {
                        const u64 x = tmp[sb + j];
                        u32 r = 0, seen = 0;
                        for (u32 m = 0; m < c; m++) {
                            const u64 y = tmp[sb + m];
                            const u32 eqb = (y == x) & (m < j);
                            r += (y < x) | eqb;
                            seen |= eqb;
                        }
                        xs[i] = x; rkb[i] = r;
                        nd += seen;
                    }
                }
                __syncthreads();
#pragma unroll
                for (int i = 0; i < SK_E; i++)
                    if (rkb[i] != 0xffffffffu) tmp[sb + rkb[i]] = xs[i];
            }
        }
    }
    if (nd) atomicAdd(&ndup_s, nd);
    __syncthreads();
    const u32 n_rep = ndup_s;
    const bool any_dup = n_rep != 0;
    const u32 n_distinct = n_kept - n_rep;
    const bool posts = A.part_keys != nullptr && B.in_lds;
    if (tid == 0 && n_rep) atomicAdd((unsigned long long *)A.drops_out, (unsigned long long)n_rep);
    SK_STAMP_AT(5);
    const u32 p0 = tid * SK_E;
    u32 rep = 0;
    u32 srl[2] = {0, 0};
    u32 rk[SK_E];
    u32 ab[SK_E / 2];
#pragma unroll
    for (int i = 0; i < SK_E / 2; i++) ab[i] = 0x00010001u;
    const bool fastp = early && !any_dup;
    if (early && any_dup) {
        if (tid < 256) bins[tid] = 0;
        __syncthreads();
    }
    if (fastp) {
        if (onerun) {
            rep = kept_mask;
            srl[0] = srl[1] = srel_one * 0x01010101u;
#pragma unroll
            for (int i = 0; i < SK_E; i++) rk[i] = (rkp[i >> 1] >> ((i & 1) * 16)) & 0xffffu;
        } else {
#pragma unroll
            for (int i = 0; i < SK_E; i++) {
                const bool kept = bo[i] != 0xffffffffu;
                rep |= (kept ? 1u : 0u) << i;
                srl[i >> 2] |= (kept ? (bo[i] >> 24) : 0u) << (8 * (i & 3));
                rk[i] = (rkp[i >> 1] >> ((i & 1) * 16)) & 0xffffu;
            }
        }
    } else
    if (any_dup || posts) {
    if ((tid & ~63u) * SK_E < n_kept) {
        {
            const uint4 a = *(const uint4 *)&tmp[p0], b = *(const uint4 *)&tmp[p0 + 2], c = *(const uint4 *)&tmp[p0 + 4],
                        d = *(const uint4 *)&tmp[p0 + 6];
            h[0] = (u64)a.x | ((u64)a.y << 32); h[1] = (u64)a.z | ((u64)a.w << 32);
            h[2] = (u64)b.x | ((u64)b.y << 32); h[3] = (u64)b.z | ((u64)b.w << 32);
            h[4] = (u64)c.x | ((u64)c.y << 32); h[5] = (u64)c.z | ((u64)c.w << 32);
            h[6] = (u64)d.x | ((u64)d.y << 32); h[7] = (u64)d.z | ((u64)d.w << 32);
        }
        const u32 nl = p0 >= n_kept ? 0u : (n_kept - p0 < SK_E ? n_kept - p0 : SK_E);
        const u32 live = (1u << nl) - 1u;
        u32 heads = 0;
        if (B.in_lds) {
            const u32 lane = tid & 63u, pw = (tid & ~63u) * SK_E;
            u32 nb4 = 0;
            {
                const uint2 dd = *(const uint2 *)&dseq[4u * lane];
                const u32 dv[4] = {dd.x & 0xffffu, dd.x >> 16, dd.y & 0xffffu, dd.y >> 16};
#pragma unroll
                for (int i = 0; i < 4; i++) {
// ... 31 lines not shown
                    const u32 mid = (lo + hi) >> 1;
                    if ((u32)dseq[mid] <= p0) lo = mid; else hi = mid;
                }
                u32 s = lo, nxt = dseq[s + 1];
#pragma unroll
                for (int i = 0; i < SK_E; i++) {
                    const u32 p = p0 + i;
                    while (p >= nxt && s + 1 < ns) { s++; nxt = dseq[s + 1]; }
                    heads |= (p == (u32)dseq[s] ? 1u : 0u) << i;
                    srl[i >> 2] |= s << (8 * (i & 3));
                }
            }
        } else {
            heads = ((const u8 *)flagbits)[tid];
        }
        rep = live;
        if (any_dup) {
            u64 prev = p0 ? tmp[p0 - 1] : 0;
            rep = 0;
#pragma unroll
            for (int i = 0; i < SK_E; i++) {
                const bool r = h[i] != prev || ((heads >> i) & 1u);
                rep |= (r ? 1u : 0u) << i;
                prev = h[i];
            }
            rep = (rep | (p0 == 0 ? 1u : 0u)) & live;
        }
    }
    if (posts) {
#pragma unroll
        for (int i = 0; i < SK_E; i++)
            if (rep & (1u << i)) rk[i] = atomicAdd(&bins[sk_digit(h[i], A.part_K, A.part_kshift, A.part_mask)], 1u);
    }
    __syncthreads();
    }

    if (any_dup) {
        ((u8 *)flagbits)[tid] = (u8)rep;
        __syncthreads();
        u32 v = tid < SK_NFLAG ? (u32)__popc(flagbits[tid]) : 0;
        u32 total;
        u32 ex = ks_block_excl_scan(v, scan_smem, &total);
        if (tid < SK_NFLAG) flagpre[tid] = ex;
        if (tid == 0) flagpre[SK_NFLAG] = total;
        if (rep) {
            u32 after = n_kept;
            for (u32 w = (p0 + SK_E) >> 5; w < SK_NFLAG; w++) {
                u32 m = flagbits[w];
                if (w == (p0 + SK_E) >> 5) m &= ~0u << ((p0 + SK_E) & 31u);
                if (m) { after = w * 32u + (u32)__builtin_ctz(m); break; }
            }
#pragma unroll
            for (int i = 0; i < SK_E; i++)
                if (rep & (1u << i)) {
                    const u32 later = rep >> (i + 1);
                    const u32 len = later ? (u32)__builtin_ctz(later) + 1u : after - (p0 + i);
                    ab[i >> 1] = (ab[i >> 1] & ~(0xffffu << ((i & 1) * 16))) | (len << ((i & 1) * 16));
                }
        }
        __syncthreads();
    }

    auto drank = [&](u32 x) -> u32 {
        if (!any_dup) return x < n_kept ? x : n_kept;
        return x >= SK_TILE ? n_distinct : flagpre[x >> 5] + (u32)__popc(flagbits[x >> 5] & ((1u << (x & 31)) - 1u));
    };
    u16 *abund_s = (u16 *)cnt;
    auto stage_reps = [&]() {
#pragma unroll
        for (int i = 0; i < SK_E; i++)
            if (rep & (1u << i)) {
                const u32 d = drank(p0 + i);
                tmp[d] = h[i];
                abund_s[d] = (u16)(ab[i >> 1] >> ((i & 1) * 16));
            }
    };
    u32 p_cnt = 0, p_off = 0;
    const u32 p_seg = (tid << A.part_sub_shift) | (blockIdx.x & ((1u << A.part_sub_shift) - 1u));
    auto post_reserve = [&]() {
        p_cnt = tid < 256 ? bins[tid] : 0;
        if (p_cnt) p_off = atomicAdd(&A.part_cursor[p_seg], p_cnt);
    };
    auto post_slices = [&]() {
        const u32 c = p_cnt, off = p_off, seg = p_seg;
        const u32 ex = sk_block_excl_scan1(c, scan_smem);
        if (tid < 256) {
            const bool fits = (u64)off + c <= A.part_cap;
            if (c && !fits) atomicOr(&A.ticket[1], 2u);
            gaddr[tid] = (fits ? (u64)seg * A.part_cap + off : A.part_cap * ((u64)(A.part_mask + 1u) << A.part_sub_shift)) - ex;
            bins[tid] = ex;
        }
    };
    auto post_emit = [&]() {
        u16 *qrel = (u16 *)cnt;
        u32 ds8[SK_E];
#pragma unroll
        for (int i = 0; i < SK_E; i++) ds8[i] = bins[sk_digit(h[i], A.part_K, A.part_kshift, A.part_mask)];
#pragma unroll
        for (int i = 0; i < SK_E; i++)
            if (rep & (1u << i)) {
                const u32 pos = ds8[i] + rk[i];
                tmp[pos] = h[i];
                qrel[pos] = (u16)((srl[i >> 2] >> (8 * (i & 3))) & 0xffu);
            }
        __syncthreads();
        for (u32 i = tid; i < n_distinct; i += SK_THREADS) {
            const u64 hh = tmp[i];
            const u64 at = gaddr[sk_digit(hh, A.part_K, A.part_kshift, A.part_mask)] + i;
#ifndef SK_NO_POST_STORES
            const u32 qid = s_first + qrel[i];
            if (A.part_s) {
                const u32 sh = A.part_s - 32u, fm = 0xffu << sh;
                const u32 hi = (((u32)(hh >> 32)) & ~fm) | ((qid << sh) & fm);
#ifdef SK_NT_POST
                __builtin_nontemporal_store(((u64)hi << 32) | (u32)hh, &A.part_keys[at]);
                __builtin_nontemporal_store((u16)(qid >> 8), &((u16 *)A.part_vals)[at]);
#else
                A.part_keys[at] = ((u64)hi << 32) | (u32)hh;
                ((u16 *)A.part_vals)[at] = (u16)(qid >> 8);
#endif
            } else {
                A.part_keys[at] = hh;
                A.part_vals[at] = qid;
            }
#else
            if (at == 0xffffffffffffULL) A.part_vals[0] = (u32)hh + qrel[i];
#endif
        }
    };

    if (MODE == 1) {
        if (tid == 0) { A.counts[s_first] = n_distinct; A.kept[s_first] = n_kept; }
        SK_STAMP_AT(6);
        if (any_dup) {
            stage_reps();
            __syncthreads();
        }
        SK_STAMP_AT(7);
        const u64 r0 = A.offs[s_first];
        for (u32 d = tid; d < n_distinct; d += SK_THREADS) {
            A.out_hash[r0 + d] = tmp[d];
            A.out_abund[r0 + d] = any_dup ? (u32)abund_s[d] : 1u;
        }
        if (posts) {
            post_reserve();
            post_slices();
            __syncthreads();
            post_emit();
        }
    } else {
        if (posts) post_reserve();
        if (B.in_lds && any_dup)
            for (u32 i = tid; i <= ns; i += SK_THREADS) dsd[i] = (u16)drank(dseq[i]);
        if (tid < ne) ext_d[tid] = B.in_lds ? (u32)dseq[ext_seq[tid] - s_first] : bstart(B.at(ext_seq[tid]));
        if (B.in_lds && any_dup) stage_reps();
        SK_STAMP_AT(6);
        u64 excl = 0;
#ifdef SK_NO_LOOKBACK
        excl = (u64)tile * 3600u;
        if (false) {
#else
        if (tile > 0) {
#endif
            const u32 lane = tid & 63u, wave = tid >> 6;
            i64 idx = (i64)tile - 1;
            ks_spin spin = ks_spin_begin();
            for (;;) {
                if (wave < SK_LB_WAVES) {
                    u64 is_pre;
                    const u64 contrib = ks_lookback_round(idx - 64 * (i64)wave, lane, ks_lookback_words(A.tile_status), spin, &A.ticket[1], &is_pre);
                    if (lane == 0) { lb_sum[wave] = contrib; lb_pre[wave] = is_pre ? 1u : 0u; }
                }
                __syncthreads();
                bool found = false;
#pragma unroll
                for (u32 w = 0; w < SK_LB_WAVES; w++)
                    if (!found) { excl += lb_sum[w]; found = lb_pre[w] != 0; }
#ifdef SK_LB_STATS
                if (tid == 0) atomicAdd((unsigned long long *)(A.drops_out + 1), 1ULL);
#endif
                if (found) break;
                idx -= 64 * SK_LB_WAVES;
                __syncthreads();
            }
            if (tid == 0 && tile != A.debug_skip_tile)
                __hip_atomic_store(&A.tile_status[tile], KS_LB_PRE | (excl + agg), __ATOMIC_RELAXED, __HIP_MEMORY_SCOPE_AGENT);
        } else {
            __syncthreads();
        }
        const u64 base = excl;
        auto krank = [&](u32 p) -> u32 { return bstart(p < SK_TILE ? p : SK_TILE); };
        for (u32 s = s_first + tid; s < s_end; s += SK_THREADS) {
            const u32 i = s - s_first;
            const u32 ls = B.at(s), le = B.at(s + 1);
            u64 pos = base + (B.in_lds ? (u32)dseq[i] : krank(ls));
            for (u32 e = 0; e < ne; e++) pos += ext_seq[e] < s ? ext_cnt[e] : 0;
            A.csr[s] = pos;
            if (!(le > A.le_cap || le - ls > A.max_len_tile)) {
                u32 c;
                if (B.in_lds) c = any_dup ? (u32)dsd[i + 1] - (u32)dsd[i] : (u32)dseq[i + 1] - (u32)dseq[i];
                else c = any_dup ? drank(krank(le)) - drank(krank(ls)) : krank(le) - krank(ls);
                A.counts[s] = c;
            }
        }
        if (s_end == A.n_seqs && tid == 0) { A.csr[A.n_seqs] = base + agg; *A.total_out = base + agg; }
        if (!B.in_lds && any_dup) {
            for (u32 s = s_first + tid; s < s_end; s += SK_THREADS) {
                const u32 ls = B.at(s), le = B.at(s + 1);
                if (le > A.le_cap || le - ls > A.max_len_tile) continue;
                u64 pos = base + krank(ls);
                for (u32 e = 0; e < ne; e++) pos += ext_seq[e] < s ? ext_cnt[e] : 0;
                const u32 b = krank(ls), e2 = krank(le);
                for (u32 p = b; p < e2;) {
                    u32 q = p + 1;
                    while (q < e2 && !((flagbits[q >> 5] >> (q & 31u)) & 1u)) q++;
                    if (pos < A.out_cap) { A.out_hash[pos] = tmp[p]; A.out_abund[pos] = q - p; }
                    pos++;
                    p = q;
                }
            }
        }
        SK_STAMP_AT(7);
        for (u32 d = tid; d < ((!B.in_lds && any_dup) ? 0u : n_distinct); d += SK_THREADS) {
            u64 pos = base + d;
            if (!any_dup) {
                for (u32 e = 0; e < ne; e++) pos += ext_d[e] <= d ? ext_cnt[e] : 0;
            } else {
                u32 lo = 0, hi = ns;
                while (hi - lo > 1) {
                    const u32 mid = (lo + hi) >> 1;
                    if ((u32)dsd[mid] <= d) lo = mid; else hi = mid;
                }
                pos = base + (u32)dseq[lo] + (d - (u32)dsd[lo]);
                for (u32 e = 0; e < ne; e++) pos += ext_seq[e] < s_first + lo ? ext_cnt[e] : 0;
            }
#ifdef SK_NO_CSR_STORES
            if (pos == 0xffffffffffffULL) A.out_abund[0] = (u32)tmp[d];
#else
            if (pos < A.out_cap) {
#ifndef SK_T_CSR
                __builtin_nontemporal_store(tmp[d], &A.out_hash[pos]);
                __builtin_nontemporal_store(any_dup ? (u32)abund_s[d] : 1u, &A.out_abund[pos]);
#else
                A.out_hash[pos] = tmp[d];
                A.out_abund[pos] = any_dup ? (u32)abund_s[d] : 1u;
#endif
            }
#endif
        }
    }
    if (MODE == 0 && posts) {
        __syncthreads();
        post_slices();
        __syncthreads();
        post_emit();
    }
    if (A.part_keys && !B.in_lds) {
        if (tid == 0) atomicOr(&A.ticket[1], 2u);
    }
    SK_STAMP_AT(8);
}

template <int MODE, int CMP, int KC>
__global__ __launch_bounds__(SK_THREADS, MODE == 1 ? 4 : SK_MINW) void k_sketch_tiles(sk_args A) {
    if (MODE == 1) {
        const u32 n = *A.n_list < A.n_list_cap ? *A.n_list : A.n_list_cap;
        for (u32 t = blockIdx.x; t < n; t += gridDim.x) {
            sk_tile_body<MODE, CMP, KC>(A, t);
            __syncthreads();
        }
    } else {
        if (A.n_tiles_dev && blockIdx.x >= *A.n_tiles_dev) return;
        sk_tile_body<MODE, CMP, KC>(A, blockIdx.x);
    }
}

__global__ __launch_bounds__(256) void k_find_long(const u64 *offs, u32 n_seqs, u32 R, u32 span, u32 *med_ids, u32 *long_ids, u32 *n_cls,
                                                   u32 med_cap, u32 long_cap) {
    const u32 s = blockIdx.x * blockDim.x + threadIdx.x;
    u32 cls = 2;
    if (s < n_seqs) {
        const u64 len = offs[s + 1] - offs[s];
        if (R == 0) { if (len > PK_MAX_LEN) cls = 1; }
        else if (len + 16 > span || sk_deferred(offs[s], len, R, span)) cls = len > SK_MED_MAX ? 1 : 0;
    }
#pragma unroll
    for (u32 c = 0; c < 2; c++) {
        const u64 m = __ballot(cls == c);
        if (m == 0) continue;
        const u32 leader = (u32)__ffsll((long long)m) - 1u;
        u32 base = 0;
        if ((threadIdx.x & 63) == leader) base = atomicAdd(&n_cls[c], (u32)__popcll(m));
        base = __shfl(base, (int)leader, 64);
        if (cls == c && base + ks_lane_lt_count(m) < (c == 0 ? med_cap : long_cap)) (c == 0 ? med_ids : long_ids)[base + ks_lane_lt_count(m)] = s;
    }
}

struct sk_cands { u32 r[SK_NR]; };
__global__ __launch_bounds__(256) void k_seq_stats(const u64 *offs, u32 n_seqs, u32 k, u32 span, sk_cands cand, u64 *out) {
    u64 w = 0, mx = 0;
    u32 npk = 0;
    u32 nd[SK_NR], nl[SK_NR];
#pragma unroll
    for (int c = 0; c < SK_NR; c++) { nd[c] = 0; nl[c] = 0; }
    for (u32 s = blockIdx.x * blockDim.x + threadIdx.x; s < n_seqs; s += gridDim.x * blockDim.x) {
        const u64 st = offs[s], len = offs[s + 1] - st;
        w += len >= k ? len - k + 1 : 0;
        mx = len > mx ? len : mx;
        npk += len > PK_MAX_LEN ? 1u : 0u;
#pragma unroll
        for (int c = 0; c < SK_NR - 2; c++)
            if (len + cand.r[c] + 15 > span) {
                const bool def = len + 16 > span || sk_deferred(st, len, cand.r[c], span);
                nd[c] += (def && len <= SK_MED_MAX) ? 1u : 0u;
                nl[c] += (def && len > SK_MED_MAX) ? 1u : 0u;
            }
    }
    for (int d = 32; d > 0; d >>= 1) {
        w += __shfl_down(w, d, 64);
        npk += __shfl_down(npk, d, 64);
        u64 o = __shfl_down(mx, d, 64);
        mx = o > mx ? o : mx;
#pragma unroll
        for (int c = 0; c < SK_NR; c++) { nd[c] += __shfl_down(nd[c], d, 64); nl[c] += __shfl_down(nl[c], d, 64); }
    }
    if ((threadIdx.x & 63) == 0 && npk) atomicAdd((unsigned long long *)&out[SK_CTL_N_PK_LONG], (unsigned long long)npk);
    __shared__ u64 red[4][2 + 2 * SK_NR];
    const u32 wave = threadIdx.x >> 6;
    if ((threadIdx.x & 63) == 0) {
        red[wave][0] = w; red[wave][1] = mx;
#pragma unroll
        for (int c = 0; c < SK_NR; c++) { red[wave][2 + c] = nd[c]; red[wave][2 + SK_NR + c] = nl[c]; }
    }
    __syncthreads();
    if (threadIdx.x < 2 + 2 * SK_NR) {
        const u32 j = threadIdx.x;
        u64 v = red[0][j];
        for (u32 q = 1; q < 4; q++) v = j == 1 ? (red[q][j] > v ? red[q][j] : v) : v + red[q][j];
        if (v) {
            if (j == 1) atomicMax((unsigned long long *)&out[SK_CTL_MAX_LEN], (unsigned long long)v);
            else atomicAdd((unsigned long long *)&out[j == 0 ? SK_CTL_WINDOWS : SK_CTL_MED + (j - 2)], (unsigned long long)v);
        }
    }
}


struct sk_call {
    const u8 *d_res;
    const u64 *d_offs;
    u32 n_seqs;
    u64 n_res;
    u32 max_seq_len;
    const ks_params *p;
};

struct sk_plan {
    bool planned;
    bool compact;
    bool packed;
    u32 c_div, span, pk_chunk, pk_chunks;
    sk_cands cand;
    u64 pk_bound;
    u64 tiles_hint;
    u32 real_max, tile_R;
    u64 n_med, n_long;
    u64 win_bound;
    u64 pk_n_tiles;
    u64 out_cap;
    int part_pbits;
    u32 part_K, part_regions, part_sub_shift, part_kshift, part_s;
    u64 part_cap;
};

static void sk_plan_shape(const ks_ctx *ctx, const sk_call &C, int variant, sk_plan *P) {
    memset(P, 0, sizeof *P);
    const ks_params *p = C.p;
    P->planned = C.max_seq_len > 0 && !ks_dbg(ctx, KS_DBG_NO_PLAN);
    P->compact = (variant & 1) && p->scaled >= 2 && !ks_dbg(ctx, KS_DBG_NO_COMPACT);
    P->c_div = P->compact ? (p->scaled < 64 ? p->scaled : 64u) : 1u;
    P->span = SK_TILE;
    if (P->compact) {
        u64 sp = (u64)P->c_div * 3840;
        if (sp > 8ull * SK_TILE) sp = 8ull * SK_TILE;
        P->span = (u32)(sp / 512 * 512);
        if (const char *f = ks_dbg(ctx, KS_DBG_SPAN)) {
            const u32 v = (u32)atoi(f) / 512 * 512;
            if (v >= SK_TILE && v <= sp) P->span = v;
        }
    }
    P->packed = !P->compact && !ks_dbg(ctx, KS_DBG_NO_PACK);
    P->pk_chunk = C.n_seqs >= 262144 ? PK_CHUNK : (C.n_seqs >= 32768 ? 256u : 64u);
    P->pk_chunks = (C.n_seqs + P->pk_chunk - 1) / P->pk_chunk;
    for (int c = 0; c < SK_NR; c++) P->cand.r[c] = sk_r_cand_host[c] + (P->span - SK_TILE);
    P->tile_R = sk_r_cand_host[0];
    if (P->packed && P->planned && C.max_seq_len <= PK_MAX_LEN && !ks_dbg(ctx, KS_DBG_PLAN_SYNC)) {
        const u64 b = C.n_res / (SK_MED_MAX - 15 - C.max_seq_len + 1) + P->pk_chunks + 1;
        const u64 typical = C.n_res / 3800 + P->pk_chunks + 1;
        if (b <= 2 * typical + 256 && b <= C.n_seqs) P->pk_bound = b;
        else if (C.n_seqs <= 2 * typical + 256) P->pk_bound = C.n_seqs;
    }
    P->tiles_hint = P->packed ? P->pk_bound : C.n_res / P->cand.r[0] + 2;
}

static bool sk_plan_reads_stats(const sk_plan &P) { return !P.pk_bound && (!P.planned || P.packed); }

static int sk_plan_stride(ks_ctx *ctx, const sk_call &C, const u64 *stats, sk_plan *P) {
    if (P->pk_bound) {
        P->real_max = C.max_seq_len;
        P->win_bound = C.n_res;
        P->tile_R = 0; P->n_med = 0; P->n_long = 0;
        P->pk_n_tiles = P->pk_bound;
    } else if (stats) {
        P->win_bound = stats[SK_CTL_WINDOWS];
        if (P->packed) P->pk_n_tiles = *(const u32 *)(stats + SK_CTL_PK_TILES);
        if (stats[SK_CTL_MAX_LEN] > 0xfffffff0ULL) return ks_fail(ctx, KS_ERR_INVALID_ARG, "sequence longer than 2^32 residues");
        P->real_max = (u32)stats[SK_CTL_MAX_LEN];
        double best = 0;
        const double per_tile = (double)P->span / SK_TILE;
        for (int c = 0; c < SK_NR; c++) {
            if (c >= SK_NR - 2 && (u64)P->real_max + P->cand.r[c] + 15 > P->span) continue;
            const double cost = (double)(C.n_res / P->cand.r[c] + 1) * per_tile + 1.75 * (double)stats[SK_CTL_MED + c] +
                                20.0 * (double)stats[SK_CTL_LONG + c];
            if (c == 0 || cost < best) { best = cost; P->tile_R = P->cand.r[c]; P->n_med = stats[SK_CTL_MED + c]; P->n_long = stats[SK_CTL_LONG + c]; }
        }
        if (const char *force = ks_dbg(ctx, KS_DBG_TILE_R))
            for (int c = 0; c < SK_NR - 2; c++)
                if (atoi(force) == (int)sk_r_cand_host[c]) { P->tile_R = P->cand.r[c]; P->n_med = stats[SK_CTL_MED + c]; P->n_long = stats[SK_CTL_LONG + c]; }
        if (P->packed) { P->tile_R = 0; P->n_med = 0; P->n_long = stats[SK_CTL_N_PK_LONG]; }
    } else {
        P->real_max = C.max_seq_len;
        P->win_bound = C.n_res;
        P->tile_R = P->cand.r[3];
        for (int c = SK_NR - 1; c >= SK_NR - 2; c--)
            if ((u64)P->real_max + P->cand.r[c] + 15 <= P->span) { P->tile_R = P->cand.r[c]; break; }
        const bool may_defer = (u64)P->real_max + P->tile_R + 15 > P->span;
        const u64 n_t = C.n_res / P->tile_R + 1;
        P->n_med = may_defer ? n_t : 0;
        P->n_long = (may_defer && P->real_max > SK_MED_MAX) ? n_t : 0;
    }
    return KS_OK;
}

static void sk_plan_outputs(const ks_ctx *ctx, const sk_call &C, int variant, int part_pbits, int part_fmt10, sk_plan *P) {
    const ks_params *p = C.p;
    const u64 n_windows = P->win_bound;
    P->out_cap = n_windows;
    if (!(variant & 2) && p->scaled >= 2) {
        const u64 want = n_windows / p->scaled + n_windows / (4ull * p->scaled) + 65536;
        if (want < P->out_cap) P->out_cap = want;
    }
    if (const char *f = ks_dbg(ctx, KS_DBG_OUT_CAP))
        if (!(variant & 2) && strtoull(f, nullptr, 10) < P->out_cap) P->out_cap = strtoull(f, nullptr, 10);
    if (!(part_pbits > 0 && n_windows > 0 && n_windows < 0xffff0000ULL)) return;
    const int dbits = part_pbits < 8 ? part_pbits : 8;
    P->part_pbits = part_pbits;
    P->part_K = ks_join_prefix_mul(part_pbits, ks_max_hash(p->scaled));
    P->part_regions = 1u << dbits;
    P->part_sub_shift = 0u;
    if (part_pbits > 8)
        while (P->part_sub_shift < 3u && (n_windows / p->scaled) >> (8u + P->part_sub_shift + 1u) >= 65536u) P->part_sub_shift++;
    if (const char *f = ks_dbg(ctx, KS_DBG_SUBSHIFT)) { const int v = atoi(f); if (part_pbits > 8 && v >= 0 && v <= 3) P->part_sub_shift = (u32)v; }
    const u32 n_segs = P->part_regions << P->part_sub_shift;
    const u64 per = n_windows / p->scaled / n_segs + 1;
    u64 cap = per + per / 4 + 8192;
    cap = (cap + 8191) / 8192 * 8192;
    P->part_cap = cap;
    P->part_kshift = (P->part_K & (P->part_K - 1)) == 0 && P->part_K > 1 ? 32u - (u32)__builtin_ctz(P->part_K) : 0u;
    if (part_fmt10 && P->part_kshift && part_pbits > 8 && C.n_seqs < (1u << 24) && !ks_dbg(ctx, KS_DBG_POSTINGS12))
        P->part_s = 32u + P->part_kshift;
}

struct sk_bufs {
    u32 *ticket, *d_ntiles;
    u32 *tile_first;
    u64 *tile_g0;
    ks_deferred def;
};

static int sk_launch_stats(ks_ctx *ctx, ks_sketches *S, const sk_call &C, const sk_plan &P, ks_scratch &sc, sk_bufs &B) {
    const size_t ctl_words = (size_t)SK_CTL_TILE_STATUS + P.tiles_hint + 1;
    KS_TRY(ks_alloc(ctx, &S->ctl_block, ctl_words));
    u64 *const ctl = S->ctl_block;
    KS_HIP(ctx, hipMemsetAsync(ctl, 0, ctl_words * sizeof(u64), ctx->stream));
    B.ticket = (u32 *)(ctl + SK_CTL_TICKET); B.def.n_cls = (u32 *)(ctl + SK_CTL_CLS); B.d_ntiles = (u32 *)(ctl + SK_CTL_PK_TILES);
    u32 g = (C.n_seqs + 1023) / 1024;
    if (g > 512) g = 512;
    KS_LAUNCH(ctx, "seq_stats", k_seq_stats, g, 256, C.d_offs, C.n_seqs, C.p->ksize, P.span, P.cand, ctl);
    if (P.packed) {
        u32 *pk_tiles = nullptr, *pk_cnt = nullptr;
        KS_TRY(sc.alloc(&pk_tiles, (size_t)C.n_seqs));
        KS_TRY(sc.alloc(&pk_cnt, (size_t)P.pk_chunks));
        KS_TRY(sc.alloc(&B.tile_first, (size_t)C.n_seqs + 1));
        KS_TRY(sc.alloc(&B.tile_g0, (size_t)C.n_seqs + 1));
        ks_timer_begin(ctx, "tile_plan");
        hipLaunchKernelGGL(k_pack_walk, dim3(P.pk_chunks), dim3(64), 0, ctx->stream, C.d_offs, C.n_seqs, P.pk_chunk, pk_tiles, pk_cnt);
        hipLaunchKernelGGL(k_pack_fill, dim3(P.pk_chunks), dim3(256), 0, ctx->stream, C.d_offs, C.n_seqs, P.pk_chunk, (const u32 *)pk_tiles,
                           (const u32 *)pk_cnt, P.pk_chunks, B.tile_first, B.tile_g0, B.d_ntiles);
        ks_timer_end(ctx);
        KS_HIP(ctx, hipGetLastError());
    }
    return KS_OK;
}

static int sk_launch_deferred(ks_ctx *ctx, const sk_call &C, const sk_plan &P, sk_args &A, ks_scratch &sc, sk_bufs &B) {
    const u64 n_med = P.n_med, n_long = P.n_long;
    KS_TRY(sc.alloc(&A.kept, (size_t)C.n_seqs));
    if (n_med + n_long > 0) {
        KS_TRY(sc.alloc(&B.def.lg_hash, (size_t)C.n_res + 1));
        KS_TRY(sc.alloc(&B.def.lg_abund, (size_t)C.n_res + 1));
        KS_TRY(sc.alloc(&B.def.med_ids, (size_t)n_med + 1));
        KS_TRY(sc.alloc(&B.def.long_ids, (size_t)n_long + 1));
        KS_LAUNCH(ctx, "find_long", k_find_long, (C.n_seqs + 255) / 256, 256, C.d_offs, C.n_seqs, P.tile_R, P.span, B.def.med_ids,
                  B.def.long_ids, B.def.n_cls, (u32)n_med, (u32)n_long);
    }
    if (n_med > 0) {
        sk_args M = A;
        M.out_hash = B.def.lg_hash; M.out_abund = B.def.lg_abund; M.le_cap = SK_TILE; M.seq_list = B.def.med_ids;
        M.out_cap = ~0ULL;
        M.n_list = B.def.n_cls; M.n_list_cap = (u32)n_med;
        KS_LAUNCH(ctx, "sketch_medium", (k_sketch_tiles<1, 0, 0>), (u32)(n_med < 2048 ? n_med : 2048), SK_THREADS, M);
    }
    if (n_long > 0) KS_TRY(ks_sketch_long_launch(ctx, A, B.def, n_long, P.real_max, sc));
    return KS_OK;
}

static int sk_launch_tiles(ks_ctx *ctx, ks_sketches *S, const sk_call &C, const sk_plan &P, sk_args &A, int allow_defer, ks_scratch &sc,
                           sk_bufs &B) {
    const u64 n_tiles = P.packed ? P.pk_n_tiles : C.n_res / P.tile_R + 1;
    if (n_tiles > 0x7ffffff0ULL) return ks_fail(ctx, KS_ERR_INVALID_ARG, "batch too large");
    unsigned long long *tile_status = (unsigned long long *)(S->ctl_block + SK_CTL_TILE_STATUS);
    if (n_tiles > P.tiles_hint) {
        KS_TRY(sc.alloc(&tile_status, (size_t)n_tiles + 1));
        KS_HIP(ctx, hipMemsetAsync(tile_status, 0, (size_t)n_tiles * sizeof(unsigned long long), ctx->stream));
    }
    if (!P.packed) {
        KS_TRY(sc.alloc(&B.tile_first, (size_t)n_tiles + 1));
        KS_LAUNCH(ctx, "tile_plan", k_tile_plan, (u32)((n_tiles + 256) / 256), 256, C.d_offs, C.n_seqs, (u32)n_tiles, P.tile_R, B.tile_first);
    }
    A.seq_list = B.tile_first; A.le_cap = P.span - 16; A.R = P.tile_R; A.span = P.span; A.tile_g0 = B.tile_g0;
    if (P.packed) A.max_len_tile = PK_MAX_LEN;
    if (P.compact) { A.c_div = P.c_div; A.c_rcp = (u32)(((1ULL << 32) + P.c_div - 1) / P.c_div); }
    A.out_hash = S->d_hashes; A.out_abund = S->d_abunds; A.csr = S->d_offsets;
    A.tile_status = tile_status; A.n_tiles = (u32)n_tiles;
    A.n_tiles_dev = P.pk_bound ? B.d_ntiles : nullptr;
    A.drops_out = S->ctl_block + SK_CTL_DROPS;
    u32 *part_snap = nullptr;
    if (A.part_cursor && P.n_med > 0) {
        KS_TRY(sc.alloc(&part_snap, 2048));
        KS_HIP(ctx, hipMemcpyAsync(part_snap, A.part_cursor, 2048 * sizeof(u32), hipMemcpyDeviceToDevice, ctx->stream));
    }
    const u64 *rb = ctx->h_pin + KS_PIN_SKETCH_SYNC;
    for (int attempt = 0; attempt < 2; attempt++) {
        A.use_ticket = (ctx->sketch_use_ticket || attempt == 1) ? 1u : 0u;
        A.debug_skip_tile = 0xffffffffu;
        if (!A.use_ticket && ks_dbg(ctx, KS_DBG_LOOKBACK_SKIP)) A.debug_skip_tile = (u32)atoi(ks_dbg(ctx, KS_DBG_LOOKBACK_SKIP));
        if (attempt == 1) {
            ctx->sketch_use_ticket = true;
            ctx->sketch_ticket_fallbacks++;
            KS_HIP(ctx, hipMemsetAsync(tile_status, 0, (size_t)n_tiles * sizeof(unsigned long long), ctx->stream));
            KS_HIP(ctx, hipMemsetAsync(A.drops_out, 0, sizeof(u64), ctx->stream));
            const u32 keep_bits = ((const u32 *)(rb + SK_CTL_TICKET))[1] & SK_ST_POSTINGS;
            KS_HIP(ctx, hipMemsetAsync(B.ticket, 0, 2 * sizeof(u32), ctx->stream));
            if (keep_bits) {
                u32 *stage = (u32 *)(ctx->h_pin + KS_PIN_STAGE);
                *stage = keep_bits;
                KS_HIP(ctx, hipMemcpyAsync(B.ticket + 1, stage, sizeof(u32), hipMemcpyHostToDevice, ctx->stream));
            }
            if (part_snap) KS_HIP(ctx, hipMemcpyAsync(A.part_cursor, part_snap, 2048 * sizeof(u32), hipMemcpyDeviceToDevice, ctx->stream));
            else if (A.part_cursor) KS_HIP(ctx, hipMemsetAsync(A.part_cursor, 0, 2048 * sizeof(u32), ctx->stream));
        }
        ks_timer_begin(ctx, "sketch_tiles");
#define SK_LAUNCH_TILES(CMP_, KC_) hipLaunchKernelGGL((k_sketch_tiles<0, CMP_, KC_>), dim3((u32)n_tiles), dim3(SK_THREADS), 0, ctx->stream, A)
        if (P.compact) {
            if (C.p->ksize == 16) SK_LAUNCH_TILES(1, 16);
            else if (C.p->ksize == 24) SK_LAUNCH_TILES(1, 24);
            else SK_LAUNCH_TILES(1, 0);
        } else {
            if (C.p->ksize == 10) SK_LAUNCH_TILES(0, 10);
            else if (C.p->ksize == 7) SK_LAUNCH_TILES(0, 7);
            else SK_LAUNCH_TILES(0, 0);
        }
#undef SK_LAUNCH_TILES
        ks_timer_end(ctx);
        KS_HIP(ctx, hipGetLastError());

        KS_TRY(ks_sketch_place_launch(ctx, A, B.def, P.n_med, P.n_long));
        if (allow_defer && attempt == 0 && (P.pk_bound || (P.planned && !P.packed)) && !ks_dbg(ctx, KS_DBG_FORCE_TICKET_RETRY)) {
            S->pend_stats = S->ctl_block;
            S->pending = 1; S->pend_out_cap = P.out_cap; S->pend_max_seq_len = C.max_seq_len; S->pend_planned = P.planned ? 1 : 0;
            S->n_hashes = S->n_slots = P.out_cap;
            return KS_OK;
        }
        {
            const ks_fetch_seg f = ks_fetch_words(S->ctl_block, ctx->h_pin + KS_PIN_SKETCH_SYNC, SK_CTL_WORDS * 2);
            KS_TRY(ks_stream_wait_fetch(ctx, &f, 1));
        }
        u32 &status_w = ((u32 *)(ctx->h_pin + KS_PIN_SKETCH_SYNC + SK_CTL_TICKET))[1];
        if (attempt == 0 && !A.use_ticket && ks_dbg(ctx, KS_DBG_FORCE_TICKET_RETRY)) status_w |= SK_ST_LOOKBACK;
        if (!(status_w & SK_ST_LOOKBACK) || A.use_ticket) break;
    }
#ifdef SK_LB_STATS
    fprintf(stderr, "[SK_LB_STATS] tiles %llu look-back rounds %llu\n", (unsigned long long)n_tiles, (unsigned long long)rb[SK_CTL_LB_ROUNDS]);
#endif
    return KS_OK;
}

enum { SK_OUT_FINE = 0, SK_OUT_COMPACT = 1, SK_OUT_CAP = 2, SK_OUT_LOOKBACK = 3, SK_OUT_POSTINGS = 4 };

static int sk_decode(ks_ctx *ctx, ks_sketches *S, const u64 *ctl, u64 out_cap, u32 max_seq_len, bool planned, int *outcome) {
    *outcome = SK_OUT_FINE;
    S->n_slots = ctl[SK_CTL_TOTAL];
    const u64 drops = ctl[SK_CTL_DROPS] + ctl[SK_CTL_DROPS_DEF];
    S->n_hashes = S->n_slots - (drops < S->n_slots ? drops : S->n_slots);
    S->gapped = S->n_hashes != S->n_slots;
    if (planned) {
        S->n_windows = ctl[SK_CTL_WINDOWS];
        if (ctl[SK_CTL_MAX_LEN] > (u64)max_seq_len)
            return ks_fail(ctx, KS_ERR_INVALID_ARG, "max_seq_len = %u, but the batch holds a sequence of %llu residues", max_seq_len,
                           (unsigned long long)ctl[SK_CTL_MAX_LEN]);
    }
    const u32 status = ((const u32 *)(ctl + SK_CTL_TICKET))[1];
    if (status & SK_ST_LOOKBACK) *outcome = SK_OUT_LOOKBACK;
    else if (status & SK_ST_COMPACT) *outcome = SK_OUT_COMPACT;
    else if (S->n_slots > out_cap) *outcome = SK_OUT_CAP;
    else if (status & SK_ST_POSTINGS) *outcome = SK_OUT_POSTINGS;
    return KS_OK;
}

static int sketch_attempt_run(ks_ctx *ctx, ks_sketches *S, const sk_call &C, int part_pbits, int part_fmt10, int variant, int allow_defer,
                              int *redo) {
    const ks_params *p = C.p;
    KS_TRY(ks_alloc(ctx, &S->d_offsets, (size_t)C.n_seqs + 1));
    KS_TRY(ks_alloc(ctx, &S->d_counts, (size_t)C.n_seqs + 1));
    if (C.n_seqs == 0) {
        KS_HIP(ctx, hipMemsetAsync(S->d_offsets, 0, sizeof(u64), ctx->stream));
        KS_TRY(ks_alloc(ctx, &S->d_hashes, 1));
        KS_TRY(ks_alloc(ctx, &S->d_abunds, 1));
        return ks_stream_wait(ctx);
    }
    sk_plan P;
    sk_plan_shape(ctx, C, variant, &P);
    ks_scratch sc(ctx);
    sk_bufs B;
    memset(&B, 0, sizeof B);
    KS_TRY(sk_launch_stats(ctx, S, C, P, sc, B));
    const u64 *stats = nullptr;
    if (sk_plan_reads_stats(P)) {
        const ks_fetch_seg f = ks_fetch_words(S->ctl_block, ctx->h_pin + KS_PIN_SKETCH_SYNC, SK_CTL_WORDS * 2);
        KS_TRY(ks_stream_wait_fetch(ctx, &f, 1));
        stats = ctx->h_pin + KS_PIN_SKETCH_SYNC;
    }
    KS_TRY(sk_plan_stride(ctx, C, stats, &P));
    S->n_windows = P.win_bound;
    sk_plan_outputs(ctx, C, variant, part_pbits, part_fmt10, &P);
    KS_TRY(ks_alloc(ctx, &S->d_hashes, (size_t)P.out_cap));
    KS_TRY(ks_alloc(ctx, &S->d_abunds, (size_t)P.out_cap));

    sk_args A;
    memset(&A, 0, sizeof A);
    A.res = C.d_res; A.offs = C.d_offs; A.n_seqs = C.n_seqs; A.n_res = C.n_res; A.k = p->ksize; A.seed = p->seed;
    A.max_hash = ks_max_hash(p->scaled);
    {
        u64 sf = (1ULL << 48) / ((A.max_hash >> 32) + 1ULL);
        A.sfix = sf > 0x7fffffffULL ? 0x7fffffffu : (u32)sf;
    }
    A.lut = ctx->d_lut + 256 * p->moltype;
    A.upper_only = p->moltype == KS_PROTEIN ? 1u : 0u;
    if (const char *f = ks_dbg(ctx, KS_DBG_QCAP)) A.debug_qcap = (u32)atoi(f);
    A.counts = S->d_counts;
    A.drops_out = S->ctl_block + SK_CTL_DROPS_DEF;
    A.span = SK_TILE; A.c_div = 1; A.c_rcp = 0; A.out_cap = P.out_cap; A.max_len_tile = 0xffffffffu; A.R = 1;
    A.ticket = B.ticket; A.total_out = S->ctl_block + SK_CTL_TOTAL;
    if (P.part_pbits) {
        S->part_pbits = P.part_pbits; S->part_K = P.part_K; S->part_regions = P.part_regions; S->part_sub_shift = P.part_sub_shift;
        S->part_cap = P.part_cap; S->part_s = P.part_s;
        const size_t n_slots = (size_t)(P.part_cap * (P.part_regions << P.part_sub_shift)) + SK_TILE;
        KS_TRY(ks_alloc(ctx, &S->part_keys, n_slots));
        KS_TRY(ks_alloc(ctx, &S->part_vals, n_slots));
        S->part_len = (u32 *)(S->ctl_block + SK_CTL_CURSORS);
        A.part_keys = S->part_keys; A.part_vals = S->part_vals; A.part_cursor = S->part_len; A.part_cap = P.part_cap;
        A.part_K = P.part_K; A.part_mask = P.part_regions - 1; A.part_sub_shift = P.part_sub_shift;
        A.part_kshift = P.part_kshift; A.part_s = P.part_s;
    }
    KS_TRY(sk_launch_deferred(ctx, C, P, A, sc, B));
    KS_TRY(sk_launch_tiles(ctx, S, C, P, A, allow_defer, sc, B));
    if (S->pending) return KS_OK;

    int outcome = SK_OUT_FINE;
    KS_TRY(sk_decode(ctx, S, ctx->h_pin + KS_PIN_SKETCH_SYNC, P.out_cap, C.max_seq_len, P.planned, &outcome));
    switch (outcome) {
    case SK_OUT_LOOKBACK: return ks_fail(ctx, KS_ERR_HIP, "sketch: tile look-back timed out");
    case SK_OUT_COMPACT:
    case SK_OUT_CAP: *redo = outcome; return KS_OK;
    case SK_OUT_POSTINGS:
        ks_pool_free(ctx, S->part_keys); ks_pool_free(ctx, S->part_vals);
        S->part_keys = nullptr; S->part_vals = nullptr; S->part_len = nullptr; S->part_pbits = 0;
        return KS_OK;
    }
    return KS_OK;
}

static int sketch_attempt(ks_ctx *ctx, const u8 *d_res, const u64 *d_offs, u32 n_seqs, u64 n_res, u32 max_seq_len, const ks_params *p,
                          int part_pbits, int part_fmt10, int variant, int allow_defer, int *redo, ks_sketches **out) {
    ks_result<ks_sketches> S(ctx, out, ks_sketches_free);
    S->params = *p;
    S->n_seqs = n_seqs;
    *redo = 0;
    const sk_call C{d_res, d_offs, n_seqs, n_res, max_seq_len, p};
    KS_TRY(sketch_attempt_run(ctx, S, C, part_pbits, part_fmt10, variant, allow_defer, redo));
    return *redo ? KS_OK : S.commit();
}

ks_fetch_seg ks_sketch_pending_seg(const ks_sketches *S) {
    return ks_fetch_words(S->pend_stats, S->ctx->h_pin + KS_PIN_SKETCH, SK_CTL_WORDS * 2);
}

int ks_sketch_finish_pending(ks_sketches *S, int *redo) {
    *redo = 0;
    if (!S || !S->pending) return KS_OK;
    S->pending = 0;
    S->pend_stats = nullptr;
    return sk_decode(S->ctx, S, S->ctx->h_pin + KS_PIN_SKETCH, S->pend_out_cap, S->pend_max_seq_len, S->pend_planned != 0, redo);
}
// ... 19 lines not shown
```

kmerseek_amd/csrc/ks_tile.h:

```cpp
#pragma once
#include "ks_device.h"

#ifndef SK_THREADS
#define SK_THREADS 512
#endif
#define SK_E 8
#define SK_TILE (SK_THREADS * SK_E)
#define SK_PAD 160
#define SK_SEQ_CAP 254

struct sk_args {
    const u8 *res;
    const u64 *offs;
    u32 n_seqs;
    u64 n_res;
    u32 k;
    u64 seed;
    u64 max_hash;
    u32 sfix;
    const u8 *lut;
    u32 upper_only;
    u32 R;
    const u64 *tile_g0;
    u32 span;
    u32 c_div, c_rcp;
    u64 out_cap;
    u32 use_ticket;
    u32 debug_qcap;
    u32 debug_skip_tile;
    u32 le_cap;
    u32 max_len_tile;
    const u32 *seq_list;
    const u32 *n_list;
    u32 n_list_cap;
    u64 *out_hash;
    u32 *out_abund;
    u64 *csr;
    u64 *total_out;
    u32 *counts;
    u32 *kept;
    u64 *drops_out;
    unsigned long long *tile_status;
    u32 *ticket;
    u32 n_tiles;
    const u32 *n_tiles_dev;
    u64 *part_keys;
    u32 *part_vals;
    u32 *part_cursor;
    u64 part_cap;
    u32 part_K, part_mask;
    u32 part_kshift;
    u32 part_s;
    u32 part_sub_shift;
};

KS_DEV u32 sk_bucket_mul(u32 nw, u32 sfix) {
    u64 m = ((u64)nw * sfix) >> 16;
    return m > 0xffffffffULL ? 0xffffffffu : (u32)m;
}

template <int I, int KC = 0>
KS_DEV u64 sk_hash_window(const u64 *w , u32 k_rt, u64 seed) {
    const u32 k = KC ? (u32)KC : k_rt;
    ks_murmur m;
    m.init(seed);
    const u32 nb = k >> 4, t = k & 15;
    u32 j = 0;
    for (u32 b = 0; b < nb; b++, j += 2) {
        u64 a0 = w[j], a1 = w[j + 1], a2 = w[j + 2];
        m.block(ks_funnel<I>(a0, a1), ks_funnel<I>(a1, a2));
    }
    if (t) {
        u64 a0 = w[j], a1 = w[j + 1], a2 = w[j + 2];
        u64 k1 = ks_funnel<I>(a0, a1), k2 = ks_funnel<I>(a1, a2);
        if (t > 8) k2 &= ks_mask_bytes(t - 8); else { k1 &= ks_mask_bytes(t); k2 = 0; }
        m.tail(k1, k2, t);
    }
    return m.finish((u64)k);
}

KS_DEV u64 sk_hash_window_rt(const u64 *w, u32 byte_shift, u32 k, u64 seed) {
    ks_murmur m;
    m.init(seed);
    const u32 nb = k >> 4, t = k & 15;
    u32 jj = 0;
    for (u32 bl = 0; bl < nb; bl++, jj += 2)
        m.block(ks_funnel_rt(w[jj], w[jj + 1], byte_shift), ks_funnel_rt(w[jj + 1], w[jj + 2], byte_shift));
    if (t) {
        u64 k1 = ks_funnel_rt(w[jj], w[jj + 1], byte_shift), k2 = ks_funnel_rt(w[jj + 1], w[jj + 2], byte_shift);
        if (t > 8) k2 &= ks_mask_bytes(t - 8); else { k1 &= ks_mask_bytes(t); k2 = 0; }
        m.tail(k1, k2, t);
    }
    return m.finish((u64)k);
}

template <int H, int NW, int KC = 0, int I = 0>
KS_DEV void sk_hash_windows(u64 *h, const u64 *w, u32 k_rt, u64 seed) {
    if constexpr (I < NW) {
        h[I] = sk_hash_window<H + I, KC>(w, k_rt, seed);
        sk_hash_windows<H, NW, KC, I + 1>(h, w, k_rt, seed);
    }
}

KS_DEV uint4 sk_load16(const u8 *res, u64 n_res, u64 g) {
#ifdef SK_NT_RES
    if (g + 16 <= n_res) { const u32 *p4 = (const u32 *)(res + g); return make_uint4(__builtin_nontemporal_load(p4), __builtin_nontemporal_load(p4 + 1), __builtin_nontemporal_load(p4 + 2), __builtin_nontemporal_load(p4 + 3)); }
#else
    if (g + 16 <= n_res) return *(const uint4 *)(res + g);
#endif
    u32 t[4] = {0, 0, 0, 0};
    for (u32 b = 0; b < 16 && g + b < n_res; b++) t[b >> 2] |= (u32)res[g + b] << (8 * (b & 3));
    return make_uint4(t[0], t[1], t[2], t[3]);
}
KS_DEV uint4 sk_encode16(uint4 v, const u8 *lut_s, bool upper_only ) {
    const u32 in[4] = {v.x, v.y, v.z, v.w};
    u32 o[4];
    if (upper_only) {
#pragma unroll
        for (int d = 0; d < 4; d++) {
            const u32 y = in[d] & 0x7f7f7f7fu;
            const u32 lower = (y + 0x1f1f1f1fu) & ~(y + 0x05050505u) & ~in[d] & 0x80808080u;
            o[d] = in[d] ^ (lower >> 2);
        }
    } else {
#pragma unroll
        for (int d = 0; d < 4; d++)
            o[d] = (u32)lut_s[in[d] & 255u] | ((u32)lut_s[(in[d] >> 8) & 255u] << 8) |
                   ((u32)lut_s[(in[d] >> 16) & 255u] << 16) | ((u32)lut_s[in[d] >> 24] << 24);
    }
    return make_uint4(o[0], o[1], o[2], o[3]);
}

template <typename EndOf>
KS_DEV u32 sk_seq_beyond(u32 lo, u32 hi, u32 key, EndOf end_of) {
    while (lo < hi) {
        const u32 mid = lo + ((hi - lo) >> 1);
        if (end_of(mid) > key) hi = mid; else lo = mid + 1;
    }
    return lo;
}
```

kmerseek_amd/engine.py:

```python
from __future__ import annotations

import contextlib
import ctypes as C
import types
from typing import Dict, List, Optional, Sequence, Tuple

import numpy as np

from . import _lib
from ._lib import ks_params

MOLTYPES = {"protein": _lib.KS_PROTEIN, "raw": _lib.KS_PROTEIN, "dayhoff": _lib.KS_DAYHOFF, "hp": _lib.KS_HP}
MOLTYPE_NAMES = {_lib.KS_PROTEIN: "protein", _lib.KS_DAYHOFF: "dayhoff", _lib.KS_HP: "hp"}
SEED = _lib.KS_SEED_DEFAULT


class KmerseekError(RuntimeError):
    def __init__(self, status: int, message: str):
        super().__init__(message)
        self.status = status


class InvalidAminoAcid(KmerseekError):

# ... 66 lines not shown
    if side not in PILEUP_SIDES:
        raise ValueError(f"side = {side!r} is neither \"query\" nor \"target\"")
    return _lib.ks_pileup_opts(_lib.KS_PILEUP_PROFILE if profile else 0, PILEUP_SIDES[side], 0)


def karlin_ungapped(matrix, freq_q, freq_t) -> Tuple[float, float, float]:
    L = _lib.load()
    m = _matrix28(matrix)
    fq = np.ascontiguousarray(freq_q, dtype=np.float64); ft = np.ascontiguousarray(freq_t, dtype=np.float64)
    if fq.shape != (_lib.KS_RSCORE_ALPHABET,) or ft.shape != (_lib.KS_RSCORE_ALPHABET,):
        raise ValueError("freq_q and freq_t must hold 28 weights each")
    lam, K, H = C.c_double(0), C.c_double(0), C.c_double(0)
    dp = C.POINTER(C.c_double)
    st = L.ks_karlin_ungapped(m.ctypes.data_as(C.POINTER(C.c_int8)) if m is not None else None, fq.ctypes.data_as(dp), ft.ctypes.data_as(dp),
                              C.byref(lam), C.byref(K), C.byref(H))
    if st != _lib.KS_OK:
        raise KmerseekError(st, "karlin_ungapped: " + (L.ks_karlin_last_error() or L.ks_status_string(st)).decode())
    return lam.value, K.value, H.value


def search_opts(min_containment: float = 0.0, abund_stats: bool = False) -> Optional[_lib.ks_search_opts]:
    if not abund_stats and min_containment == 0.0:
        return None
    return _lib.ks_search_opts(_lib.KS_SEARCH_ABUND_STATS if abund_stats else 0, 0, float(min_containment))


def mask_opts(window: int = 12, k1: float = 2.2, k2: float = 2.5) -> _lib.ks_mask_opts:
    if _int_in("window", window, _lib.KS_MASK_MAX_WINDOW, f"[2, {_lib.KS_MASK_MAX_WINDOW}]") < 2:
        raise ValueError(f"window = {window} is not an integer in [2, {_lib.KS_MASK_MAX_WINDOW}]")
    return _lib.ks_mask_opts(int(window), _int_in("k1 in millibits", round(1000 * k1), 2 ** 32 - 1),
                             _int_in("k2 in millibits", round(1000 * k2), 2 ** 32 - 1))


BEST_RANK_BY = {"intersect": _lib.KS_BEST_INTERSECT, "target_containment": _lib.KS_BEST_TARGET_CONTAINMENT,
                "max_containment": _lib.KS_BEST_MAX_CONTAINMENT, "jaccard": _lib.KS_BEST_JACCARD, "score": _lib.KS_BEST_SCORE}
GREEDY_ASSIGN = {"first": _lib.KS_GREEDY_ASSIGN_FIRST, "best": _lib.KS_GREEDY_ASSIGN_BEST}


class _FollowDebugEnv:

    def __init__(self, L, ctx):
        self._L, self._ctx = L, ctx

    def __getattr__(self, name):
        f = getattr(self._L, name)
        if not name.startswith("ks_") or name in ("ks_ctx_create", "ks_ctx_destroy", "ks_ctx_reload_debug_env", "ks_last_error",
                                                    "ks_status_string"):
            return f

        def call(*a):
            if self._ctx._h:
                self._L.ks_ctx_reload_debug_env(self._ctx._h)
            return f(*a)
        return call


class Context:

    _HIP_STREAM_LEGACY = 1

    def __init__(self, device: int = 0, stream: Optional[int] = None, follow_debug_env: bool = False):
        self._L = _lib.load()
        self._h = None
        if follow_debug_env:
            self._L = _FollowDebugEnv(self._L, self)
        h = C.c_void_p()
        sp = None if stream is None else C.c_void_p(int(stream) if int(stream) != 0 else self._HIP_STREAM_LEGACY)
        st = self._L.ks_ctx_create(int(device), sp, C.byref(h))
        if st != _lib.KS_OK:
            raise KmerseekError(st, f"ks_ctx_create(device={device}) failed: {self._L.ks_status_string(st).decode()}"
                                    " — the HIP path has no CPU fallback")
        self._h = h
        self.device = device
        self._pinned, self._close_pending = 0, False

    def close(self):
        if getattr(self, "_pinned", 0) > 0:
            self._close_pending = True
            return
        if getattr(self, "_h", None):
            self._L.ks_ctx_destroy(self._h)
            self._h = None

    def __del__(self):
        try:
            self.close()
        except Exception:
            pass

    def __enter__(self):
        return self

    def __exit__(self, *a):
        self.close()

    def _check(self, st: int):
        if st != _lib.KS_OK:
            msg = self._L.ks_last_error(self._h).decode() or self._L.ks_status_string(st).decode()
            raise KmerseekError(st, msg)

    @property
    def stream(self) -> int:
        v = int(self._L.ks_ctx_stream(self._h) or 0)
        return 0 if v == self._HIP_STREAM_LEGACY else v

    def synchronize(self):
        self._check(self._L.ks_ctx_synchronize(self._h))

    def to_device(self, a: np.ndarray) -> "DeviceBuffer":
        a = np.ascontiguousarray(a)
        p = C.c_void_p()
        self._check(self._L.ks_dev_malloc(self._h, a.nbytes, C.byref(p)))
        buf = DeviceBuffer(self, p, a.nbytes)
        self._check(self._L.ks_dev_upload(self._h, p, _ptr(a), a.nbytes))
        return buf

    @contextlib.contextmanager
    def _uploaded(self, *arrays):
        bufs = []
        try:
            for a in arrays:
                bufs.append(self.to_device(a))
            yield [b.ptr for b in bufs]
        finally:
            for b in bufs:
                b.free()

    @contextlib.contextmanager
    def _batches(self, q_res, q_off, t_res, t_off):
        q_res = np.ascontiguousarray(q_res, dtype=np.uint8); q_off = np.ascontiguousarray(q_off, dtype=np.uint64)
        t_res = np.ascontiguousarray(t_res, dtype=np.uint8); t_off = np.ascontiguousarray(t_off, dtype=np.uint64)
        with self._uploaded(q_res, q_off, t_res, t_off) as (d_q, d_qo, d_t, d_to):
            yield d_q, d_qo, len(q_off) - 1, len(q_res), d_t, d_to, len(t_off) - 1, len(t_res)

    def _device_empty(self, nbytes: int) -> "DeviceBuffer":
        p = C.c_void_p()
        self._check(self._L.ks_dev_malloc(self._h, int(nbytes), C.byref(p)))
        return DeviceBuffer(self, p, int(nbytes))

    def pinned_empty(self, n: int, dtype) -> np.ndarray:
        dt = np.dtype(dtype)
        nbytes = max(int(n) * dt.itemsize, 1)
        p = C.c_void_p()
        self._check(self._L.ks_host_alloc(self._h, nbytes, C.byref(p)))
        buf = (C.c_char * nbytes).from_address(p.value)
        buf._owner = _PinnedBlock(self, p)
        return np.frombuffer(buf, dtype=dt, count=int(n))

    def pool_stats(self) -> Dict[str, int]:
        v = [C.c_uint64(0) for _ in range(4)]
        self._check(self._L.ks_ctx_pool_stats(self._h, *[C.byref(x) for x in v]))
        return dict(zip(("blocks", "bytes_held", "bytes_in_use", "mallocs"), (int(x.value) for x in v)))

    def sketch_stats(self) -> Dict[str, int]:
        v = (C.c_uint64 * 4)()
        self._check(self._L.ks_ctx_sketch_stats(self._h, C.byref(v)))
        return {"ticket_fallbacks": int(v[0]), "uses_ticket": int(v[1]), "compact_fallbacks": int(v[2]), "cap_fallbacks": int(v[3])}

    def unpack_hits64_device(self, d_packed: int, n: int, qbits: int, tbits: int, d_qid: int, d_tid: int, d_isect: int, d_nw: int):
        self._check(self._L.ks_hits_unpack64_device(self._h, C.c_void_p(d_packed), n, qbits, tbits, C.c_void_p(d_qid), C.c_void_p(d_tid),
                                                    C.c_void_p(d_isect), C.c_void_p(d_nw)))

    def merge_hits_by_qid_device(self, d_qid: int, d_tid: int, d_isect: int, d_nw: int, block_rows: Sequence[int], n_queries: int,
                                 o_qid: int, o_tid: int, o_isect: int, o_nw: int):
        rows = (C.c_uint64 * len(block_rows))(*[int(x) for x in block_rows])
        self._check(self._L.ks_hits_merge_by_qid_device(self._h, C.c_void_p(d_qid), C.c_void_p(d_tid), C.c_void_p(d_isect), C.c_void_p(d_nw),
                                                        rows, len(block_rows), int(n_queries), C.c_void_p(o_qid), C.c_void_p(o_tid),
                                                        C.c_void_p(o_isect), C.c_void_p(o_nw)))

    def reload_debug_env(self):
        self._check(self._L.ks_ctx_reload_debug_env(self._h))

    def search_stats(self, paths: bool = False) -> Dict[str, int]:
        v = (C.c_uint64 * 5)()
        self._check(self._L.ks_ctx_search_stats(self._h, C.byref(v)))
        out = {"join_retries": int(v[0]), "rows_ticket_fallbacks": int(v[1]), "agg_overflows": int(v[3])}
        if paths:
            out["agg_used"] = int(v[2])
            out["join_table"] = int(v[4])
        return out

    def debug_scan(self, kind: int, d_in: int, d_out: int, n: int, d_total: int = 0):
        self._check(self._L.ks_debug_scan(self._h, int(kind), C.c_void_p(d_in), C.c_void_p(d_out), int(n), C.c_void_p(d_total or None)))

    def debug_scan_seek(self, global_tile: int):
        self._check(self._L.ks_debug_scan_seek(self._h, int(global_tile) & 0xffffffff))

    def debug_scan_ticket(self) -> int:
        v = C.c_uint32(0)
        self._check(self._L.ks_debug_scan_ticket(self._h, C.byref(v)))
        return int(v.value)

    def debug_radix_sort(self, vbytes: int, d_keys: int, d_vals: int, n: int, shifts: Sequence[int], d_keys_out: int, d_vals_out: int,
                         pfx_k: int = 0, d_seg_len: int = 0, seg_cap: int = 0, seg_regions: int = 0, alias_in: bool = False):
        sh = (C.c_int * max(len(shifts), 1))(*[int(s) for s in shifts])
        self._check(self._L.ks_debug_radix_sort(self._h, int(vbytes), C.c_void_p(d_keys), C.c_void_p(d_vals or None), int(n), sh, len(shifts),
                                                int(pfx_k), C.c_void_p(d_seg_len or None), int(seg_cap), int(seg_regions), int(bool(alias_in)),
                                                C.c_void_p(d_keys_out), C.c_void_p(d_vals_out or None)))

    def debug_msd_sort(self, d_keys: int, n: int, lo_bit: int, nbits: int, seg_count: Optional[Sequence[int]] = None,
                       seg_cap: int = 0) -> Dict[str, int]:
        info = (C.c_uint32 * 4)()
        sc = None if seg_count is None else (C.c_uint32 * max(len(seg_count), 1))(*[int(c) for c in seg_count])
        self._check(self._L.ks_debug_msd_sort(self._h, C.c_void_p(d_keys), int(n), int(lo_bit), int(nbits), sc,
                                              0 if seg_count is None else len(seg_count), int(seg_cap), C.byref(info)))
        return dict(zip(("done", "bits2", "n_buckets", "big"), (int(x) for x in info)))

    def sketch_batch(self, residues: np.ndarray, offsets: np.ndarray, ksize: int, scaled: int, moltype: str,
                     seed: int = SEED) -> "Sketches":
        residues = np.ascontiguousarray(residues, dtype=np.uint8)
        offsets = np.ascontiguousarray(offsets, dtype=np.uint64)
        p = make_params(ksize, scaled, moltype, seed)
        out = C.c_void_p()
        self._check(self._L.ks_sketch_batch(self._h, _ptr(residues), _ptr(offsets), len(offsets) - 1, C.byref(p),
                                            C.byref(out)))
        return Sketches(self, out)

    def sketch_batch_device(self, d_residues: int, d_offsets: int, n_seqs: int, n_residues: int, ksize: int,
                            scaled: int, moltype: str, max_seq_len: int = 0, seed: int = SEED) -> "Sketches":
        p = make_params(ksize, scaled, moltype, seed)
        out = C.c_void_p()
        self._check(self._L.ks_sketch_batch_device(self._h, C.c_void_p(d_residues), C.c_void_p(d_offsets), n_seqs,
                                                   n_residues, max_seq_len, C.byref(p), C.byref(out)))
        return Sketches(self, out)

    def sketch_queries_device(self, index: "Index", d_residues: int, d_offsets: int, n_seqs: int, n_residues: int,
                              max_seq_len: int = 0) -> "Sketches":
        out = C.c_void_p()
        self._check(self._L.ks_sketch_queries_device(self._h, index._h, C.c_void_p(d_residues), C.c_void_p(d_offsets),
                                                     n_seqs, n_residues, max_seq_len, C.byref(out)))
        return Sketches(self, out)

    def sketch_search_device(self, index: "Index", d_residues: int, d_offsets: int, n_seqs: int, n_residues: int,
                             max_seq_len: int = 0, want_sketches: bool = True, *, min_containment: float = 0.0,
                             abund_stats: bool = False):
        sk, hits = C.c_void_p(), C.c_void_p()
        opts = search_opts(min_containment, abund_stats)
        if opts is None:
            st = self._L.ks_sketch_search_device(self._h, index._h, C.c_void_p(d_residues), C.c_void_p(d_offsets), n_seqs,
                                                 n_residues, max_seq_len, C.byref(sk) if want_sketches else None, C.byref(hits))
        else:
            st = self._L.ks_sketch_search_device_ex(self._h, index._h, C.c_void_p(d_residues), C.c_void_p(d_offsets), n_seqs,
                                                    n_residues, max_seq_len, C.byref(opts), C.byref(sk) if want_sketches else None,
                                                    C.byref(hits))
        self._check(st)
        return (Sketches(self, sk) if want_sketches else None), Hits(self, hits)

    def sketch_search(self, index: "Index", residues: np.ndarray, offsets: np.ndarray, want_sketches: bool = True, *,
                      min_containment: float = 0.0, abund_stats: bool = False):
        residues = np.ascontiguousarray(residues, dtype=np.uint8)
        offsets = np.ascontiguousarray(offsets, dtype=np.uint64)
        sk, hits = C.c_void_p(), C.c_void_p()
        opts = search_opts(min_containment, abund_stats)
        if opts is None:
            st = self._L.ks_sketch_search(self._h, index._h, _ptr(residues), _ptr(offsets), len(offsets) - 1,
                                          C.byref(sk) if want_sketches else None, C.byref(hits))
        else:
            st = self._L.ks_sketch_search_ex(self._h, index._h, _ptr(residues), _ptr(offsets), len(offsets) - 1, C.byref(opts),
                                             C.byref(sk) if want_sketches else None, C.byref(hits))
        self._check(st)
        return (Sketches(self, sk) if want_sketches else None), Hits(self, hits)

    def translate6(self, nt: np.ndarray, offsets: np.ndarray) -> Tuple["DeviceBuffer", "DeviceBuffer", int]:
        nt = np.ascontiguousarray(nt, dtype=np.uint8)
        offsets = np.ascontiguousarray(offsets, dtype=np.uint64)
        n, n_nt = len(offsets) - 1, int(offsets[-1])
        if nt.size != n_nt:
            raise ValueError(f"offsets end at {n_nt}, the batch holds {nt.size} bases")
        d_nt = self.to_device(nt if n_nt else np.zeros(16, np.uint8))
        d_off = self.to_device(offsets)
        frames = self._device_empty(int(self._L.ks_translate6_bound(n_nt)) + 16)
        foff = self._device_empty(8 * (6 * n + 1))
        n_res = C.c_uint64(0)
        try:
            self._check(self._L.ks_translate6_device(self._h, d_nt._p, d_off._p, n, n_nt, frames._p, foff._p, C.byref(n_res)))
        finally:
            d_nt.free(); d_off.free()
        return frames, foff, int(n_res.value)

    def sketch_translated(self, nt: np.ndarray, offsets: np.ndarray, ksize: int, scaled: int, moltype: str,
                          seed: int = SEED) -> "Sketches":
        nt = np.ascontiguousarray(nt, dtype=np.uint8)
        offsets = np.ascontiguousarray(offsets, dtype=np.uint64)
        p = make_params(ksize, scaled, moltype, seed)
        out = C.c_void_p()
        self._check(self._L.ks_sketch_translated(self._h, _ptr(nt), _ptr(offsets), len(offsets) - 1, C.byref(p), C.byref(out)))
        return Sketches(self, out)

    def sketch_translated_device(self, d_nt: int, d_offsets: int, n_seqs: int, n_nt: int, ksize: int, scaled: int, moltype: str,
                                 max_seq_len: int = 0, seed: int = SEED) -> "Sketches":
        p = make_params(ksize, scaled, moltype, seed)
        out = C.c_void_p()
        self._check(self._L.ks_sketch_translated_device(self._h, C.c_void_p(d_nt), C.c_void_p(d_offsets), n_seqs, n_nt, max_seq_len,
                                                        C.byref(p), C.byref(out)))
        return Sketches(self, out)

    def mask_low_complexity(self, residues: np.ndarray, offsets: np.ndarray, window: int = 12, k1: float = 2.2, k2: float = 2.5) -> "Mask":
        residues = np.ascontiguousarray(residues, dtype=np.uint8)
        offsets = np.ascontiguousarray(offsets, dtype=np.uint64)
        o = mask_opts(window, k1, k2)
        out = C.c_void_p()
        self._check(self._L.ks_mask_batch(self._h, _ptr(residues), _ptr(offsets), len(offsets) - 1, C.byref(o), C.byref(out)))
        return Mask(self, out)

    def mask_low_complexity_device(self, d_residues: int, d_offsets: int, n_seqs: int, n_residues: int, window: int = 12, k1: float = 2.2,
                                   k2: float = 2.5) -> "Mask":
        o = mask_opts(window, k1, k2)
        out = C.c_void_p()
        self._check(self._L.ks_mask_device(self._h, C.c_void_p(d_residues), C.c_void_p(d_offsets), n_seqs, n_residues, C.byref(o), C.byref(out)))
        return Mask(self, out)
# ... 1144 lines not shown
```

Measured before the change: 63.09 billion.

## Precompute per-tile output slots in pack planner to skip decoupled lookback

When scaled is 1 (every hash kept) and the layout is packed, the pack walk kernel now also computes each sequence's window count and an exclusive prefix. This gives every tile a fixed output base, so the sketch kernel no longer needs the decoupled lookback across tiles or the tile_status memset. Windows whose hash is zero are reported through the existing extension/drop mechanism so the fixed slots stay consistent. The pack walk moves from one wave to 256 threads with a per-thread binary search and also takes over the seq_stats reductions. The cost is extra planner work and buffers, plus more complex edge-case handling that falls back to the ticket path.

```diff
diff --git a/include/kmerseek_amd.h b/include/kmerseek_amd.h
--- a/include/kmerseek_amd.h
+++ b/include/kmerseek_amd.h
@@ -63,7 +63,7 @@
 int ks_ctx_pool_stats(const ks_ctx *ctx, uint64_t *n_blocks, uint64_t *bytes_held, uint64_t *bytes_in_use,
                       uint64_t *n_mallocs);
 
-int ks_ctx_sketch_stats(const ks_ctx *ctx, uint64_t out[4]);
+int ks_ctx_sketch_stats(const ks_ctx *ctx, uint64_t out[5]);
 int ks_ctx_search_stats(const ks_ctx *ctx, uint64_t out[5]);
 int ks_ctx_fused_stats(const ks_ctx *ctx, uint64_t out[4]);
 int ks_ctx_qfilter_stats(const ks_ctx *ctx, uint64_t out[2]);
diff --git a/kmerseek_amd/_lib.py b/kmerseek_amd/_lib.py
--- a/kmerseek_amd/_lib.py
+++ b/kmerseek_amd/_lib.py
@@ -186,7 +186,7 @@
     "ks_last_error": (C.c_char_p, [_vp]),
     "ks_ctx_stream": (_vp, [_vp]),
     "ks_ctx_synchronize": (C.c_int, [_vp]),
-    "ks_ctx_sketch_stats": (C.c_int, [_vp, C.POINTER(C.c_uint64 * 4)]),
+    "ks_ctx_sketch_stats": (C.c_int, [_vp, C.POINTER(C.c_uint64 * 5)]),
     "ks_ctx_search_stats": (C.c_int, [_vp, C.POINTER(C.c_uint64 * 5)]),
     "ks_ctx_fused_stats": (C.c_int, [_vp, C.POINTER(C.c_uint64 * 4)]),
     "ks_ctx_qfilter_stats": (C.c_int, [_vp, C.POINTER(C.c_uint64 * 2)]),
diff --git a/kmerseek_amd/csrc/ks_common.h b/kmerseek_amd/csrc/ks_common.h
--- a/kmerseek_amd/csrc/ks_common.h
+++ b/kmerseek_amd/csrc/ks_common.h
@@ -40,7 +40,7 @@
     X(STAGED_H2D) X(PLAIN_COPIES) X(PAIRS_LSD) X(MSD_LDS_CAP) X(SCAN_3PASS) X(INDEX_LSD) X(JOIN_FP) X(FP_COARSEN)        \
     X(PAIR_LIMIT) X(PBITS_MAX) X(RECORD_BITS) X(ONE_CURSOR) X(JOIN_SEGS) X(JOIN_SEG_CAP) X(JOIN_SPARSE)                \
     X(NO_ROWS_HINT) X(ROWS_TICKET) X(FORCE_ROWS_TICKET_RETRY) X(FORCE_TICKET_RETRY) X(NO_PLAN) X(NO_COMPACT) X(SPAN)      \
-    X(NO_PACK) X(PLAN_SYNC) X(TILE_R) X(OUT_CAP) X(POOL_CAP) X(THROW) X(QCAP) X(LOOKBACK_SKIP) X(SYNC_API) X(POSTINGS12) X(POSTINGS10) X(NO_DEFER) X(BUCKET) X(JOIN_SPLIT) X(SUBSHIFT) X(MATCHPOS_ROW_BITS) X(SIGNIF_WAVE_ROWS) X(BEST_PATH) X(REGIONS_ROW_BITS) X(QFILTER) X(QFILTER_OCC) X(CLUSTER_PATH) X(GATHER_PATH) X(GREEDY_PATH) X(UNION_PATH) X(AGG_CAP) X(ROWS_PATH) X(CULL_PATH) X(CHAIN_PATH) X(COMP_PATH) X(PILEUP_PATH)
+    X(NO_PACK) X(PLAN_SYNC) X(TILE_R) X(OUT_CAP) X(POOL_CAP) X(THROW) X(QCAP) X(LOOKBACK_SKIP) X(TILE_LOOKBACK) X(SYNC_API) X(POSTINGS12) X(POSTINGS10) X(NO_DEFER) X(BUCKET) X(JOIN_SPLIT) X(SUBSHIFT) X(MATCHPOS_ROW_BITS) X(SIGNIF_WAVE_ROWS) X(BEST_PATH) X(REGIONS_ROW_BITS) X(QFILTER) X(QFILTER_OCC) X(CLUSTER_PATH) X(GATHER_PATH) X(GREEDY_PATH) X(UNION_PATH) X(AGG_CAP) X(ROWS_PATH) X(CULL_PATH) X(CHAIN_PATH) X(COMP_PATH) X(PILEUP_PATH)
 enum ks_dbg_id {
 #define KS_DBG_ENUM(n) KS_DBG_##n,
     KS_DBG_LIST(KS_DBG_ENUM)
@@ -76,6 +76,7 @@
     u64 rows_hint = 0;
     bool sketch_use_ticket = false;
     u64 sketch_ticket_fallbacks = 0, sketch_compact_fallbacks = 0, sketch_cap_fallbacks = 0;
+    u64 sketch_planned_slots = 0;
     bool rows_use_ticket = false; u64 rows_ticket_fallbacks = 0;
     u64 fused_deferred = 0, fused_redos = 0;
     u64 fused_aggregated = 0;
diff --git a/kmerseek_amd/csrc/ks_ctx.hip b/kmerseek_amd/csrc/ks_ctx.hip
--- a/kmerseek_amd/csrc/ks_ctx.hip
+++ b/kmerseek_amd/csrc/ks_ctx.hip
@@ -194,11 +194,12 @@
     });
 }
 
-extern "C" int ks_ctx_sketch_stats(const ks_ctx *ctx, uint64_t out[4]) {
+extern "C" int ks_ctx_sketch_stats(const ks_ctx *ctx, uint64_t out[5]) {
     return ks_guard((ks_ctx *)ctx, [&]() -> int {
     if (!ctx || !out) return KS_ERR_INVALID_ARG;
     out[0] = ctx->sketch_ticket_fallbacks; out[1] = ctx->sketch_use_ticket ? 1 : 0;
     out[2] = ctx->sketch_compact_fallbacks; out[3] = ctx->sketch_cap_fallbacks;
+    out[4] = ctx->sketch_planned_slots;
     return KS_OK;
     });
 }
diff --git a/kmerseek_amd/csrc/ks_sketch.hip b/kmerseek_amd/csrc/ks_sketch.hip
--- a/kmerseek_amd/csrc/ks_sketch.hip
+++ b/kmerseek_amd/csrc/ks_sketch.hip
@@ -128,9 +128,11 @@
     q.ok = q.nw > 0;
 }
 
-KS_DEV u32 sk_place_window(const sk_args &A, u32 p, u64 h, sk_seq &q, const sk_bounds &B, u32 s_end, u32 *cnt) {
+KS_DEV u32 sk_place_window(const sk_args &A, u32 p, u64 h, sk_seq &q, const sk_bounds &B, u32 s_end, u32 *cnt, bool *zero) {
     while (q.s < s_end && p >= q.le) { q.s++; sk_load_seq(q, A, B, s_end); }
-    const bool keep = q.ok && p >= q.ls && p + A.k <= q.le && h != 0 && h <= A.max_hash;
+    const bool real = q.ok && p >= q.ls && p + A.k <= q.le;
+    const bool keep = real && h != 0 && h <= A.max_hash;
+    *zero = real && h == 0;
     u32 bo = 0xffffffffu;
     if (keep) {
         const u32 b = q.ls + __umulhi((u32)(h >> 32), q.mul);
@@ -144,56 +146,145 @@
 
 
 #define PK_CHUNK 1024
+#define PK_THREADS 256
 #define PK_MAX_LEN (SK_MED_MAX - 16)
 
-__global__ __launch_bounds__(64) void k_pack_walk(const u64 *offs, u32 n_seqs, u32 chunk ,
-                                                  u32 *chunk_tiles , u32 *chunk_cnt) {
+KS_DEV u64 pk_block_excl_scan64(u64 v, u64 *smem, u64 *total) {
+    const u32 lane = threadIdx.x & 63, wave = threadIdx.x >> 6;
+    u64 incl = v;
+#pragma unroll
+    for (int d = 1; d < 64; d <<= 1) {
+        const u64 o = (u64)__shfl_up((unsigned long long)incl, d, 64);
+        if (lane >= (u32)d) incl += o;
+    }
+    if (lane == 63) smem[wave] = incl;
+    __syncthreads();
+    u64 base = 0, tot = 0;
+#pragma unroll
+    for (u32 w = 0; w < PK_THREADS / 64; w++) {
+        const u64 x = smem[w];
+        base += w < wave ? x : 0;
+        tot += x;
+    }
+    *total = tot;
+    return base + incl - v;
+}
+
+__global__ __launch_bounds__(PK_THREADS) void k_pack_walk(const u64 *offs, u32 n_seqs, u32 chunk , u32 k,
+                                                          u32 *chunk_tiles ,
+                                                          u64 *chunk_wb ,
+                                                          u32 *chunk_cnt, u64 *chunk_win ,
+                                                          u64 *ctl ) {
+    static_assert(PK_CHUNK % PK_THREADS == 0 && PK_CHUNK <= 0xffff, "sequences per thread; 16-bit links");
+    constexpr u32 PER = PK_CHUNK / PK_THREADS;
     __shared__ u64 lo_s[PK_CHUNK + 1];
-    const u32 lane = threadIdx.x;
+    __shared__ u64 wp_s[PK_CHUNK];
+    __shared__ u16 nxt_s[PK_CHUNK];
+    __shared__ u16 tl_s[PK_CHUNK];
+    __shared__ u64 scan_s[PK_THREADS / 64];
+    __shared__ u64 mx_s[PK_THREADS / 64];
+    __shared__ u32 npk_s[PK_THREADS / 64];
+    __shared__ u32 nt_s;
+    const u32 tid = threadIdx.x;
     const u32 c0 = blockIdx.x * chunk;
     const u32 n = (n_seqs - c0) < chunk ? (n_seqs - c0) : chunk;
-    for (u32 i = lane; i <= n; i += 64) lo_s[i] = offs[c0 + i];
-    __builtin_amdgcn_wave_barrier();
-    u32 s = 0, nt = 0;
-    while (s < n) {
-        const u64 limit = (lo_s[s] & ~15ULL) + SK_MED_MAX;
-        u32 lo = s, hi = n + 1;
-        while (hi - lo > 1) {
-            const u32 step = (hi - lo + 63) / 64;
-            const u32 idx = lo + (lane + 1) * step;
-            const bool ok = idx < hi && lo_s[idx] <= limit;
-            const u64 m = __ballot(ok);
-            const u32 good = m == ~0ULL ? 64u : (u32)__builtin_ctzll(~m);
-            const u32 nlo = lo + good * step;
-            const u32 nhi = lo + (good + 1) * step;
-            lo = nlo < hi ? nlo : hi - 1;
-            hi = nhi < hi ? nhi : hi;
-        }
-        u32 e = lo;
-        if (e == s) e = s + 1;
-        else if (e < n && lo_s[e + 1] - lo_s[e] > PK_MAX_LEN) e++;
-        if (lane == 0) chunk_tiles[c0 + nt] = c0 + s;
-        nt++;
-        s = e;
-    }
-    if (lane == 0) chunk_cnt[blockIdx.x] = nt;
-}
-
-__global__ __launch_bounds__(256) void k_pack_fill(const u64 *offs, u32 n_seqs, u32 chunk, const u32 *chunk_tiles, const u32 *chunk_cnt, u32 n_chunks,
-                                                   u32 *tile_first, u64 *tile_g0, u32 *n_tiles_out) {
+    {
+        u64 v[PER];
+#pragma unroll
+        for (u32 j = 0; j < PER; j++) {
+            const u32 i = tid + j * PK_THREADS;
+            v[j] = i <= n ? offs[c0 + i] : 0;
+        }
+        const u64 vn = tid == 0 ? offs[c0 + n] : 0;
+#pragma unroll
+        for (u32 j = 0; j < PER; j++) {
+            const u32 i = tid + j * PK_THREADS;
+            if (i <= n) lo_s[i] = v[j];
+        }
+        if (tid == 0) lo_s[n] = vn;
+    }
+    __syncthreads();
+    u64 mx = 0;
+    u32 npk = 0;
+#pragma unroll
+    for (u32 j = 0; j < PER; j++) {
+        const u32 i = tid + j * PK_THREADS;
+        u64 len = 0;
+        if (i < n) {
+            const u64 st = lo_s[i];
+            len = lo_s[i + 1] - st;
+            wp_s[i] = len >= k ? len - k + 1 : 0;
+            const u64 limit = (st & ~15ULL) + SK_MED_MAX;
+            u32 lo = i, hi = n + 1;
+            while (hi - lo > 1) {
+                const u32 mid = (lo + hi) >> 1;
+                if (lo_s[mid] <= limit) lo = mid; else hi = mid;
+            }
+            u32 e = lo;
+            if (e == i) e = i + 1;
+            else if (e < n && lo_s[e + 1] - lo_s[e] > PK_MAX_LEN) e++;
+            nxt_s[i] = (u16)e;
+        }
+        mx = len > mx ? len : mx;
+        npk += (u32)__popcll(__ballot(len > PK_MAX_LEN));
+    }
+    mx = ks_wave_max64(mx);
+    if ((tid & 63u) == 0) { mx_s[tid >> 6] = mx; npk_s[tid >> 6] = npk; }
+    __syncthreads();
+    if (tid == 0) {
+        u32 s = 0, nt = 0;
+        while (s < n) { tl_s[nt++] = (u16)s; s = nxt_s[s]; }
+        nt_s = nt;
+    }
+    if (tid == 64) {
+        u64 m = 0;
+        u32 c = 0;
+        for (u32 w = 0; w < PK_THREADS / 64; w++) { m = mx_s[w] > m ? mx_s[w] : m; c += npk_s[w]; }
+        if (m) atomicMax((unsigned long long *)&ctl[SK_CTL_MAX_LEN], (unsigned long long)m);
+        if (c) atomicAdd((unsigned long long *)&ctl[SK_CTL_N_PK_LONG], (unsigned long long)c);
+    }
+    u64 w[PER], part = 0;
+#pragma unroll
+    for (u32 j = 0; j < PER; j++) { w[j] = tid * PER + j < n ? wp_s[tid * PER + j] : 0; part += w[j]; }
+    u64 total;
+    u64 ex = pk_block_excl_scan64(part, scan_s, &total);
+#pragma unroll
+    for (u32 j = 0; j < PER; j++) { if (tid * PER + j < n) wp_s[tid * PER + j] = ex; ex += w[j]; }
+    __syncthreads();
+    const u32 nt = nt_s;
+    for (u32 i = tid; i < nt; i += PK_THREADS) {
+        const u32 s = tl_s[i];
+        chunk_tiles[c0 + i] = c0 + s;
+        chunk_wb[c0 + i] = wp_s[s];
+    }
+    if (tid == 0) { chunk_cnt[blockIdx.x] = nt; chunk_win[blockIdx.x] = total; }
+}
+
+__global__ __launch_bounds__(256) void k_pack_fill(const u64 *offs, u32 n_seqs, u32 chunk, const u32 *chunk_tiles, const u64 *chunk_wb,
+                                                   const u32 *chunk_cnt, const u64 *chunk_win, u32 n_chunks, u32 *tile_first, u64 *tile_g0,
+                                                   u64 *tile_wbase, u32 *n_tiles_out, u64 *ctl) {
     __shared__ u32 scan_smem[256 / 64 + 1];
+    __shared__ u64 win_s[256 / 64];
     u32 part = 0;
-    for (u32 c = threadIdx.x; c < blockIdx.x; c += 256) part += chunk_cnt[c];
+    u64 wpart = 0;
+    for (u32 c = threadIdx.x; c < blockIdx.x; c += 256) { part += chunk_cnt[c]; wpart += chunk_win[c]; }
+    wpart = ks_wave_sum64(wpart);
+    if ((threadIdx.x & 63u) == 0) win_s[threadIdx.x >> 6] = wpart;
     u32 total;
     (void)ks_block_excl_scan(part, scan_smem, &total);
+    u64 wbase = 0;
+    for (u32 w = 0; w < 256 / 64; w++) wbase += win_s[w];
     const u32 base = total, mine = chunk_cnt[blockIdx.x];
     for (u32 i = threadIdx.x; i < mine; i += 256) {
         const u32 sf = chunk_tiles[blockIdx.x * chunk + i];
         tile_first[base + i] = sf;
         tile_g0[base + i] = offs[sf] & ~15ULL;
+        tile_wbase[base + i] = wbase + chunk_wb[blockIdx.x * chunk + i];
     }
     if (blockIdx.x == n_chunks - 1 && threadIdx.x == 0) {
         tile_first[base + mine] = n_seqs;
+        tile_wbase[base + mine] = wbase + chunk_win[blockIdx.x];
+        ctl[SK_CTL_WINDOWS] = wbase + chunk_win[blockIdx.x];
         *n_tiles_out = base + mine;
     }
 }
@@ -307,13 +398,14 @@
     tile = (u32)__builtin_amdgcn_readfirstlane((int)tile);
     u64 g0p = 0;
     if (packed) g0p = A.tile_g0[tile];
+    const bool planned = MODE == 0 && !CMP && A.tile_wbase != nullptr;
     u32 s_first, s_end;
     if (MODE == 1) { s_first = A.seq_list[tile]; s_end = s_first + 1; }
     else { s_first = A.seq_list[tile]; s_end = A.seq_list[tile + 1]; }
     if (!A.upper_only && tid < 256) lut_s[tid] = (u8)lut_v;
     if (MODE == 0 && tid < NCH) rv = sk_load16(A.res, A.n_res, (packed ? g0p : (u64)tile * A.R) + (u64)tid * 16);
     if (s_first >= s_end) {
-        if (MODE == 0 && tid == 0)
+        if (MODE == 0 && tid == 0 && !planned)
             __hip_atomic_store(&A.tile_status[tile], KS_LB_AGG | 0ULL, __ATOMIC_RELAXED, __HIP_MEMORY_SCOPE_AGENT);
         return;
     }
@@ -360,6 +452,12 @@
 #endif
     u32 rkp[SK_E / 2] = {0, 0, 0, 0};
     u32 kept_mask = 0, srel_one = 0;
+    auto note_zero = [&](u32 s, u32 n) {
+        const u32 e = atomicAdd(&ext_n, 1u);
+        if (e < 4) { ext_seq[e] = s; ext_cnt[e] = n; ext_d[e] = 1; }
+        else atomicOr(&A.ticket[1], SK_ST_LOOKBACK);
+        atomicAdd((unsigned long long *)A.drops_out, (unsigned long long)n);
+    };
     if (CMP) {
         u8 *slist = (u8 *)cnt;
         const u32 lane = tid & 63u;
@@ -436,10 +534,12 @@
             const u32 s24 = (srel < 254u ? srel : 254u) << 24;
             const bool thr = A.max_hash != ~0ULL;
             u32 bb[SK_E], rt[SK_E];
-            u32 kpm = 0;
+            u32 kpm = 0, zm = 0;
 #pragma unroll
             for (int i = 0; i < SK_E; i++) {
-                bool keep = (q0 + (u32)i - q.ls) < q.nw && h[i] != 0;
+                const bool real = (q0 + (u32)i - q.ls) < q.nw;
+                bool keep = real && h[i] != 0;
+                zm |= (real && !keep) ? (1u << i) : 0u;
                 if (thr) keep = keep && h[i] <= A.max_hash;
                 kpm |= keep ? (1u << i) : 0u;
                 const u32 b = q.ls + __umulhi((u32)(h[i] >> 32), q.mul);
@@ -452,9 +552,20 @@
             for (int i = 0; i < SK_E; i++)
                 bo[i] = ((kpm >> i) & 1u) ? (s24 | (bb[i] << 12) | __builtin_amdgcn_ubfe(rt[i], bb[i] << 4, 16u)) : 0xffffffffu;
             kept_mask = kpm; srel_one = s24 >> 24;
+            if (planned && zm) note_zero(q.s, (u32)__popc(zm));
         } else {
-#pragma unroll
-            for (int i = 0; i < SK_E; i++) bo[i] = sk_place_window(A, q0 + i, h[i], q, B, s_end, cnt);
+            u32 zm = 0;
+#pragma unroll
+            for (int i = 0; i < SK_E; i++) {
+                bool zero;
+                bo[i] = sk_place_window(A, q0 + i, h[i], q, B, s_end, cnt, &zero);
+                zm |= zero ? (1u << i) : 0u;
+            }
+            while (planned && zm) {
+                const u32 i = (u32)__builtin_ctz(zm);
+                zm &= zm - 1u;
+                note_zero(sk_seq_beyond(s_first, s_end, q0 + i, [&](u32 s) { return B.at(s + 1); }), 1u);
+            }
         }
         if (early) {
             if (A.part_kshift) {
@@ -485,7 +596,15 @@
             const u32 ls = B.at(s), le = B.at(s + 1);
             if (le > A.le_cap || le - ls > A.max_len_tile) {
                 const u32 e = atomicAdd(&ext_n, 1u);
-                if (e < 4) { ext_seq[e] = s; ext_cnt[e] = A.kept[s]; ext_d[e] = 0; }
+                u32 c = A.kept[s];
+                if (planned) {
+                    const u64 len = A.offs[s + 1] - A.offs[s];
+                    const u32 nw = len >= A.k ? (u32)(len - A.k + 1) : 0u;
+                    if (nw != c) atomicAdd((unsigned long long *)A.drops_out, (unsigned long long)(nw - c));
+                    c = nw;
+                }
+                if (e < 4) { ext_seq[e] = s; ext_cnt[e] = c; ext_d[e] = 0; }
+                else if (planned) atomicOr(&A.ticket[1], SK_ST_LOOKBACK);
             }
         }
     }
@@ -545,8 +664,13 @@
     const u32 ne = MODE == 0 ? (ext_n < 4 ? ext_n : 4) : 0;
     u64 agg = n_kept;
     for (u32 e = 0; e < ne; e++) agg += ext_cnt[e];
-    if (MODE == 0 && tid == 0 && tile != A.debug_skip_tile)
+    if (MODE == 0 && !planned && tid == 0 && tile != A.debug_skip_tile)
         __hip_atomic_store(&A.tile_status[tile], (tile == 0 ? KS_LB_PRE : KS_LB_AGG) | agg, __ATOMIC_RELAXED, __HIP_MEMORY_SCOPE_AGENT);
+    u64 wbase = 0;
+    if (planned) {
+        const u64 wb = __builtin_nontemporal_load(&A.tile_wbase[tile]);
+        wbase = ((u64)(u32)__builtin_amdgcn_readfirstlane((int)(u32)(wb >> 32)) << 32) | (u32)__builtin_amdgcn_readfirstlane((int)(u32)wb);
+    }
 
     SK_STAMP_AT(3);
     {
@@ -884,7 +1008,11 @@
         if (posts) post_reserve();
         if (B.in_lds && any_dup)
             for (u32 i = tid; i <= ns; i += SK_THREADS) dsd[i] = (u16)drank(dseq[i]);
-        if (tid < ne) ext_d[tid] = B.in_lds ? (u32)dseq[ext_seq[tid] - s_first] : bstart(B.at(ext_seq[tid]));
+        if (tid < ne) {
+            const u32 sx = ext_seq[tid] + ext_d[tid];
+            const u32 lx = B.in_lds ? 0u : B.at(sx);
+            ext_d[tid] = B.in_lds ? (u32)dseq[sx - s_first] : bstart(lx < SK_TILE ? lx : SK_TILE);
+        }
         if (B.in_lds && any_dup) stage_reps();
         SK_STAMP_AT(6);
         u64 excl = 0;
@@ -892,6 +1020,10 @@
         excl = (u64)tile * 3600u;
         if (false) {
 #else
+        if (planned) {
+            excl = wbase;
+            __syncthreads();
+        } else
         if (tile > 0) {
 #endif
             const u32 lane = tid & 63u, wave = tid >> 6;
@@ -1090,6 +1222,7 @@
     bool planned;
     bool compact;
     bool packed;
+    bool slots;
     u32 c_div, span, pk_chunk, pk_chunks;
     sk_cands cand;
     u64 pk_bound;
@@ -1121,6 +1254,8 @@
         }
     }
     P->packed = !P->compact && !ks_dbg(ctx, KS_DBG_NO_PACK);
+    P->slots = P->packed && ks_max_hash(p->scaled) == ~0ULL && !ks_dbg(ctx, KS_DBG_TILE_LOOKBACK) && !ks_dbg(ctx, KS_DBG_LOOKBACK_SKIP) &&
+               !ks_dbg(ctx, KS_DBG_FORCE_TICKET_RETRY);
     P->pk_chunk = C.n_seqs >= 262144 ? PK_CHUNK : (C.n_seqs >= 32768 ? 256u : 64u);
     P->pk_chunks = (C.n_seqs + P->pk_chunk - 1) / P->pk_chunk;
     for (int c = 0; c < SK_NR; c++) P->cand.r[c] = sk_r_cand_host[c] + (P->span - SK_TILE);
@@ -1205,7 +1340,7 @@
 struct sk_bufs {
     u32 *ticket, *d_ntiles;
     u32 *tile_first;
-    u64 *tile_g0;
+    u64 *tile_g0, *tile_wbase;
     ks_deferred def;
 };
 
@@ -1213,21 +1348,28 @@
     const size_t ctl_words = (size_t)SK_CTL_TILE_STATUS + P.tiles_hint + 1;
     KS_TRY(ks_alloc(ctx, &S->ctl_block, ctl_words));
     u64 *const ctl = S->ctl_block;
-    KS_HIP(ctx, hipMemsetAsync(ctl, 0, ctl_words * sizeof(u64), ctx->stream));
+    KS_HIP(ctx, hipMemsetAsync(ctl, 0, (P.slots ? (size_t)SK_CTL_TILE_STATUS : ctl_words) * sizeof(u64), ctx->stream));
     B.ticket = (u32 *)(ctl + SK_CTL_TICKET); B.def.n_cls = (u32 *)(ctl + SK_CTL_CLS); B.d_ntiles = (u32 *)(ctl + SK_CTL_PK_TILES);
-    u32 g = (C.n_seqs + 1023) / 1024;
-    if (g > 512) g = 512;
-    KS_LAUNCH(ctx, "seq_stats", k_seq_stats, g, 256, C.d_offs, C.n_seqs, C.p->ksize, P.span, P.cand, ctl);
-    if (P.packed) {
+    if (!P.packed) {
+        u32 g = (C.n_seqs + 1023) / 1024;
+        if (g > 512) g = 512;
+        KS_LAUNCH(ctx, "seq_stats", k_seq_stats, g, 256, C.d_offs, C.n_seqs, C.p->ksize, P.span, P.cand, ctl);
+    } else {
         u32 *pk_tiles = nullptr, *pk_cnt = nullptr;
+        u64 *pk_wb = nullptr, *pk_win = nullptr;
         KS_TRY(sc.alloc(&pk_tiles, (size_t)C.n_seqs));
+        KS_TRY(sc.alloc(&pk_wb, (size_t)C.n_seqs));
         KS_TRY(sc.alloc(&pk_cnt, (size_t)P.pk_chunks));
+        KS_TRY(sc.alloc(&pk_win, (size_t)P.pk_chunks));
         KS_TRY(sc.alloc(&B.tile_first, (size_t)C.n_seqs + 1));
         KS_TRY(sc.alloc(&B.tile_g0, (size_t)C.n_seqs + 1));
+        KS_TRY(sc.alloc(&B.tile_wbase, (size_t)C.n_seqs + 1));
         ks_timer_begin(ctx, "tile_plan");
-        hipLaunchKernelGGL(k_pack_walk, dim3(P.pk_chunks), dim3(64), 0, ctx->stream, C.d_offs, C.n_seqs, P.pk_chunk, pk_tiles, pk_cnt);
+        hipLaunchKernelGGL(k_pack_walk, dim3(P.pk_chunks), dim3(PK_THREADS), 0, ctx->stream, C.d_offs, C.n_seqs, P.pk_chunk, C.p->ksize, pk_tiles,
+                           pk_wb, pk_cnt, pk_win, ctl);
         hipLaunchKernelGGL(k_pack_fill, dim3(P.pk_chunks), dim3(256), 0, ctx->stream, C.d_offs, C.n_seqs, P.pk_chunk, (const u32 *)pk_tiles,
-                           (const u32 *)pk_cnt, P.pk_chunks, B.tile_first, B.tile_g0, B.d_ntiles);
+                           (const u64 *)pk_wb, (const u32 *)pk_cnt, (const u64 *)pk_win, P.pk_chunks, B.tile_first, B.tile_g0, B.tile_wbase,
+                           B.d_ntiles, ctl);
         ks_timer_end(ctx);
         KS_HIP(ctx, hipGetLastError());
     }
@@ -1263,7 +1405,7 @@
     unsigned long long *tile_status = (unsigned long long *)(S->ctl_block + SK_CTL_TILE_STATUS);
     if (n_tiles > P.tiles_hint) {
         KS_TRY(sc.alloc(&tile_status, (size_t)n_tiles + 1));
-        KS_HIP(ctx, hipMemsetAsync(tile_status, 0, (size_t)n_tiles * sizeof(unsigned long long), ctx->stream));
+        if (!P.slots) KS_HIP(ctx, hipMemsetAsync(tile_status, 0, (size_t)n_tiles * sizeof(unsigned long long), ctx->stream));
     }
     if (!P.packed) {
         KS_TRY(sc.alloc(&B.tile_first, (size_t)n_tiles + 1));
@@ -1283,12 +1425,16 @@
     }
     const u64 *rb = ctx->h_pin + KS_PIN_SKETCH_SYNC;
     for (int attempt = 0; attempt < 2; attempt++) {
-        A.use_ticket = (ctx->sketch_use_ticket || attempt == 1) ? 1u : 0u;
+        const bool slots = P.slots && attempt == 0;
+        A.tile_wbase = slots ? B.tile_wbase : nullptr;
+        A.use_ticket = (!slots && (ctx->sketch_use_ticket || attempt == 1)) ? 1u : 0u;
         A.debug_skip_tile = 0xffffffffu;
         if (!A.use_ticket && ks_dbg(ctx, KS_DBG_LOOKBACK_SKIP)) A.debug_skip_tile = (u32)atoi(ks_dbg(ctx, KS_DBG_LOOKBACK_SKIP));
         if (attempt == 1) {
-            ctx->sketch_use_ticket = true;
-            ctx->sketch_ticket_fallbacks++;
+            if (!P.slots) {
+                ctx->sketch_use_ticket = true;
+                ctx->sketch_ticket_fallbacks++;
+            }
             KS_HIP(ctx, hipMemsetAsync(tile_status, 0, (size_t)n_tiles * sizeof(unsigned long long), ctx->stream));
             KS_HIP(ctx, hipMemsetAsync(A.drops_out, 0, sizeof(u64), ctx->stream));
             const u32 keep_bits = ((const u32 *)(rb + SK_CTL_TICKET))[1] & SK_ST_POSTINGS;
@@ -1301,6 +1447,7 @@
             if (part_snap) KS_HIP(ctx, hipMemcpyAsync(A.part_cursor, part_snap, 2048 * sizeof(u32), hipMemcpyDeviceToDevice, ctx->stream));
             else if (A.part_cursor) KS_HIP(ctx, hipMemsetAsync(A.part_cursor, 0, 2048 * sizeof(u32), ctx->stream));
         }
+        if (slots) ctx->sketch_planned_slots++;
         ks_timer_begin(ctx, "sketch_tiles");
 #define SK_LAUNCH_TILES(CMP_, KC_) hipLaunchKernelGGL((k_sketch_tiles<0, CMP_, KC_>), dim3((u32)n_tiles), dim3(SK_THREADS), 0, ctx->stream, A)
         if (P.compact) {
diff --git a/kmerseek_amd/csrc/ks_tile.h b/kmerseek_amd/csrc/ks_tile.h
--- a/kmerseek_amd/csrc/ks_tile.h
+++ b/kmerseek_amd/csrc/ks_tile.h
@@ -22,6 +22,7 @@
     u32 upper_only;
     u32 R;
     const u64 *tile_g0;
+    const u64 *tile_wbase;
     u32 span;
     u32 c_div, c_rcp;
     u64 out_cap;
diff --git a/kmerseek_amd/engine.py b/kmerseek_amd/engine.py
--- a/kmerseek_amd/engine.py
+++ b/kmerseek_amd/engine.py
@@ -242,10 +242,13 @@
         self._check(self._L.ks_ctx_pool_stats(self._h, *[C.byref(x) for x in v]))
         return dict(zip(("blocks", "bytes_held", "bytes_in_use", "mallocs"), (int(x.value) for x in v)))
 
-    def sketch_stats(self) -> Dict[str, int]:
-        v = (C.c_uint64 * 4)()
+    def sketch_stats(self, paths: bool = False) -> Dict[str, int]:
+        v = (C.c_uint64 * 5)()
         self._check(self._L.ks_ctx_sketch_stats(self._h, C.byref(v)))
-        return {"ticket_fallbacks": int(v[0]), "uses_ticket": int(v[1]), "compact_fallbacks": int(v[2]), "cap_fallbacks": int(v[3])}
+        out = {"ticket_fallbacks": int(v[0]), "uses_ticket": int(v[1]), "compact_fallbacks": int(v[2]), "cap_fallbacks": int(v[3])}
+        if paths:
+            out["planned_slots"] = int(v[4])
+        return out
 
     def unpack_hits64_device(self, d_packed: int, n: int, qbits: int, tbits: int, d_qid: int, d_tid: int, d_isect: int, d_nw: int):
         self._check(self._L.ks_hits_unpack64_device(self._h, C.c_void_p(d_packed), n, qbits, tbits, C.c_void_p(d_qid), C.c_void_p(d_tid),
```

New measurement: 64.30 billion, median of 6. 1.02x the previous value.
